# hvasbath/beat

Measured on AMD Instinct MI355X. Metric: SMC chain-steps/s (FFI seismic gfstacking 400 patches x 64 targets x 4096 samples), higher is better.
Workload: dtype f64; 1 GPU; BASELINE configs[2]: FFI seismic gfstacking, 400 patches x 64 targets x 4096 samples, library (64,400,3,25,4096) f64 = 62.9 GB in HBM, nearest_neighbor, covariance scalar; population SURVEY 8(d): nucleation U over the 20x20 fault, time 0; chains_per_gpu=512, global_chains=512, parallelism=chains sharded over 1 GPU(s), library replicated

## Files before the change

### beat_amd/csrc/ctx.hpp

```cpp
#pragma once
#include <hip/hip_runtime.h>

#include <cstdarg>
#include <cstdint>
#include <cstdio>
#include <cstring>
#include <map>
#include <memory>
#include <string>
#include <vector>

#include "../../include/beat_amd.h"

struct beatamd_ctx;

namespace beatamd {

void set_error(const char *fmt, ...);

#define BA_HIP(expr)                                                                         \
    do {                                                                                     \
        hipError_t e_ = (expr);                                                              \
        if (e_ != hipSuccess) {                                                              \
            beatamd::set_error("%s:%d: %s -> %s", __FILE__, __LINE__, #expr,                 \
// ... 170 lines not shown
    std::vector<int64_t> sizes;
    std::vector<int32_t> wsets;
    DevMem<int64_t> hp_off;
    bool corr_set = false;
    GeoCorr corr;
    DevMem<GeoCorrTerm> corr_terms;
    DevMem<double> corr_basis;
    DevMem<PoleTerm> pole_terms;
    mutable DevMem<double> pole_coef;
    mutable int64_t pole_chains = 0;
};

struct GeomSources {
    int nsrc = 0;
    DevMem<int32_t> kind;
    DevMem<int64_t> poff;
    DevMem<double> pfix;
    DevMem<double> east, north, los;
    int64_t Nobs = 0;
    double nu = 0.25;
};

constexpr int POL_MTQT = 0, POL_MT = 1, POL_DC = 2;
constexpr int POL_MAX_MAPS = 8;
struct PolSource {
    int32_t kind = POL_MTQT, pad_ = 0;
    int64_t off[6] = {-1, -1, -1, -1, -1, -1};
    double fix[6] = {0, 0, 0, 0, 0, 0};
};
struct Polarity {
    PolSource src;
    int32_t nmap = 0;
    int64_t NT = 0;
    int64_t map_end[POL_MAX_MAPS] = {};
    int64_t hp_off[POL_MAX_MAPS] = {};
    double hp_fix[POL_MAX_MAPS] = {};
    double gamma = 0.2;
    DevMem<double> rw, obs;
    int32_t ntab = 0;
    DevMem<double> utab, btab;
};

struct FfiModel {
    beatamd_ffi_layout layout;
    int32_t nsub = 0;
    std::vector<int32_t> ndip, nstrike, patch_off;
    std::vector<double> patch_size;
    int64_t P = 0;
    DevMem<int32_t> d_ndip, d_nstrike, d_patch_off;
    DevMem<double> d_patch_size;
    std::vector<Wavemap> wavemaps;
    bool has_geo = false;
    Geodetic geo;
    bool geo_is_geometry = false;
    GeomSources geom;
    bool has_pol = false;
    Polarity pol;
    int32_t lap = -1;
    int64_t nllk() const;
    bool obs_quads_valid = false;
    std::vector<double> obs_quads;
    DevMem<double> d_obs_quads;
    int32_t lsq_var = -1, lsq_zero_var = -1;
    bool lsq_blocks_valid = false;
    DevMem<double> lsq_GG, lsq_LtL;
};

struct HyperModel {
    int64_t nterm = 0, nh = 0;
    DevMem<double> M, slog;
    DevMem<int32_t> kind, hp_index;
    int32_t ngroups = 0, group_end[8] = {0, 0, 0, 0, 0, 0, 0, 0};
};

constexpr int KNOB_UNSET = -2147483647;
#define BEATAMD_GF_KNOBS(X) \
    X(gf_kernel, "BEATAMD_GF_KERNEL") X(gs_cg, "BEATAMD_GS_CG") X(gs_ws, "BEATAMD_GS_WS") X(gs_dma, "BEATAMD_GS_DMA") X(gs_nt, "BEATAMD_GS_NT") \
    X(ws_map, "BEATAMD_WS_MAP") X(gs_pair, "BEATAMD_GS_PAIR") X(gs_nthint, "BEATAMD_GS_NTHINT") X(gs_order, "BEATAMD_GS_ORDER") \
    X(gs_fit, "BEATAMD_GS_FIT") X(gs_win, "BEATAMD_GS_WIN") X(gf_tinv, "BEATAMD_GF_TINV") X(gs_tune, "BEATAMD_GS_TUNE") \
    X(gf_order, "BEATAMD_GF_ORDER") X(gf_cgroup, "BEATAMD_GF_CGROUP") X(gs_ml, "BEATAMD_GS_ML") X(gc_global, "BEATAMD_GC_GLOBAL") \
    X(gc_sort, "BEATAMD_GC_SORT") X(gc_keys, "BEATAMD_GC_KEYS") X(gc_bands, "BEATAMD_GC_BANDS") X(gr_cap, "BEATAMD_GR_CAP") \
    X(gr_pass_alloc, "BEATAMD_GR_PASS_ALLOC") X(gr_var, "BEATAMD_GR_VAR") X(sweep_v1, "BEATAMD_SWEEP_V1") X(qf_band, "BEATAMD_QF_BAND") \
    X(qf_fuse, "BEATAMD_QF_FUSE") X(gf_split, "BEATAMD_GF_SPLIT") X(gm_wave, "BEATAMD_GM_WAVE") X(skip_parked, "BEATAMD_SKIP_PARKED") \
    X(td_strip, "BEATAMD_TD_STRIP") X(pd_strip, "BEATAMD_PD_STRIP") X(pd_rows, "BEATAMD_PD_ROWS")
struct GfKnobs {
#define X(member, env) int member = KNOB_UNSET;
    BEATAMD_GF_KNOBS(X)
#undef X
    void read_env();
    static int get(int v, int dflt) { return v == KNOB_UNSET ? dflt : v; }
    static bool is(int v, int x) { return v != KNOB_UNSET && v == x; }
    static bool set(int v) { return v != KNOB_UNSET; }
};

struct KTimer {
    double total_ms = 0;
    int64_t n = 0;
    std::vector<std::pair<hipEvent_t, hipEvent_t>> pending;
};

}

struct beatamd_ctx {
    int device = 0;
    hipStream_t stream = nullptr, own_stream = nullptr;
    bool timing = false;
    std::map<std::string, beatamd::KTimer> timers;
    std::vector<hipEvent_t> event_pool;
    int *d_status = nullptr;
    std::vector<beatamd::DevBuf> scratch_bufs;
    std::vector<std::unique_ptr<beatamd::SeisStore>> seislibs;
    std::vector<std::unique_ptr<beatamd::GeoLib>> geolibs;
    std::vector<std::unique_ptr<beatamd::GeoEnsemble>> geoens;
    std::vector<std::unique_ptr<beatamd::WeightSet>> wsets;
    std::vector<std::unique_ptr<beatamd::Laplacian>> laps;
    std::vector<std::unique_ptr<beatamd::FfiModel>> models;
    std::vector<std::unique_ptr<beatamd::HyperModel>> hypers;
    int num_cu = 256;
    char last_gf_kernel[96] = "";
    int64_t gs_ngtp = 0, gs_N = 0;
    double gs_trep = 1;
    int gs_nvar = 1;
    bool gs_has_passes = false;
    char gf_plan[384] = "";
    char gf_tune_log[512] = "";
    uint32_t *h_umax = nullptr;
    hipEvent_t umax_event = nullptr;
    bool umax_pending = false;
    int umax_hist = -1, umax_hist_cg = 0;
    std::map<std::vector<int64_t>, std::pair<int, int>> gs_tuned;
    int gs_cg = 0;
    beatamd::GfKnobs knobs;
    bool knobs_live = false;
    uint32_t *step_dev = nullptr;
    std::map<int64_t, beatamd::DevMem<double>> twiddles;

    int get_scratch(int slot, size_t bytes, void **out);
    template <class T>
    int scratch(int slot, size_t n, T **out)
    {
        void *raw = nullptr;
        const int rc = get_scratch(slot, n * sizeof(T), &raw);
        *out = static_cast<T *>(raw);
        return rc;
    }
    hipEvent_t get_event();
    void time_begin(const char *name);
    void time_end(const char *name);
    int check_status();
};

namespace beatamd {

bool is_device_ptr(const void *p);
const GfKnobs &gf_knobs(beatamd_ctx *ctx);

enum Slot : int {
    SL_IN0 = 0, SL_IN1, SL_IN2, SL_IN3, SL_IN4, SL_IN5, SL_IN6, SL_IN7,
    SL_OUT0, SL_OUT1, SL_OUT2, SL_OUT3, SL_OUT4, SL_OUT5, SL_OUT6, SL_OUT7,
    SL_ROWOFF, SL_WEIGHTS, SL_ST0, SL_RESID, SL_PARTIAL, SL_PARTIAL2, SL_QUAD, SL_MU, SL_SLIPS,
    SL_QPROP, SL_LPROP, SL_MISC, SL_GS_UROWS, SL_GS_UCOUNT, SL_GS_SLOT, SL_GS_W, SL_GS_UMAX, SL_GS_USLOT,
    SL_CHAINBAD, SL_Z, SL_ROWSCALE, SL_CUM, SL_STAGE2, SL_WHITEN,
    SL_CHOL_A, SL_CHOL_X, SL_CHOL_D, SL_CHOL_T, SL_CHOL_L,
    SL_GC_ORDER, SL_GS_ORDER, SL_GC_STREAM, SL_GC_HDR, SL_GC_META, SL_DELTA, SL_LOGU, SL_EDGES, SL_TSLOT, SL_SPLIT, SL_WS_PACK,
    SL_GM_W, SL_GM_SCALE, SL_GM_FLAG, SL_LSQ_N, SL_LSQ_B, SL_LSQ_X, SL_LSQ_U, SL_MR_SPANS,
    SL_RES_GG, SL_RES_N, SL_RES_W, SL_RES_T, SL_RES_U, SL_RATE_DMIN, SL_SPEC,
    SL_MG_FLAG, SL_MG_MOM, SL_MG_PAR, SL_MG_GRID, SL_MG_W, SL_MG_BOX,
    SL_MC_FLAG, SL_MC_COUNT, SL_MC_SUM, SL_PD_BOX,
    SL_CV_W, SL_CV_SA, SL_CV_SB, SL_CV_Q, SL_CV_CM, SL_CV_RM, SL_CV_OFF, SL_CV_ESS, SL_CV_ACT, SL_CV_STATE, SL_CV_MAC0, SL_CV_MAC1,
    SL_CV_AC, SL_CV_RHO, SL_CV_PART, SL_COUNT
};
constexpr int SL_NIN = SL_OUT0 - SL_IN0, SL_NOUT = SL_ROWOFF - SL_OUT0;

class Staging {
    beatamd_ctx *ctx;
    int nin = 0, nout = 0, nback = 0;
    struct { void *host, *dev; size_t bytes; } back[SL_NOUT];
    int in_bytes(const void *p, size_t bytes, const void **dev);
    int out_bytes(void *p, size_t bytes, void **dev, bool preload);

public:
    explicit Staging(beatamd_ctx *c) : ctx(c) {}
    template <class T>
    int in(const T *p, size_t n, const T **dev)
    {
        const void *d = nullptr;
        BA_TRY(in_bytes(p, n * sizeof(T), &d));
        *dev = static_cast<const T *>(d);
        return BEATAMD_OK;
    }
    template <class T>
    int out(T *p, size_t n, T **dev, bool preload = false)
    {
        void *d = nullptr;
        BA_TRY(out_bytes(p, n * sizeof(T), &d, preload));
        *dev = static_cast<T *>(d);
        return BEATAMD_OK;
    }
    int finish();
};

struct ScopedTimer {
    beatamd_ctx *c;
    const char *n;
    ScopedTimer(beatamd_ctx *ctx, const char *name) : c(ctx), n(name) { c->time_begin(n); }
    ~ScopedTimer() { c->time_end(n); }
};

}
```

### beat_amd/csrc/gfshared.hip

```cpp
#include "kernels.hpp"
#include "misfit.hpp"
#include "wave.hpp"

namespace beatamd {

constexpr int GS_NT_MAX = 64;
constexpr int GS_NTHINT_DEFAULT = 1;
constexpr int GS_WS_DEFAULT = 1;

struct GroupTabArgs {
    int nrow, nvar, CG;
    int64_t C, T, P, DS;
    const uint32_t *rowoff;
    const double *fac;
    ChainVec slips[4];
    int ucap, ustride;
    uint32_t *urows;
    uint32_t *uent;
    int nissue;
    int windowed;
    int depth;
    uint32_t *ucount;
    uint32_t *umax;
    uint16_t *slot;
// ... 1441 lines not shown
    *ucap_out = (int)std::max<int64_t>(ucap, 2);
    return true;
}

GfGroup gfstack_group(const GfPlan &p, int cg, int ucap)
{
    GfGroup g;
    g.cg = cg; g.ucap = ucap;
    g.ws = p.ws512 && cg == WS_CG;
    g.mode = p.mode;
    if (p.mode == GF_RESID_BAND1) g.band1 = gf_band1(g.ws && !p.f32 && !p.pair64 && p.fused, GF_BY_WS, &g.mode);
    return g;
}

bool gfstack_shared_plan(const GfStackCall &k, GfPlan &p)
{
    const SeisLib &L = *k.libs[0];
    if (L.N % 2 != 0) return false;
    const GfKnobs &kn = *p.knobs;
    if (GfKnobs::is(kn.gf_kernel, 0)) return false;
    if (!GfKnobs::is(kn.gf_kernel, 1) && k.C < 48) return false;
    p.ws512 = GfKnobs::get(kn.gs_ws, GS_WS_DEFAULT) != 0 && k.interp != BEATAMD_MULTILINEAR && L.N % 2 == 0 &&
              !(GfKnobs::set(kn.gs_dma) && kn.gs_dma != 2) && !(GfKnobs::set(kn.gs_nt) && kn.gs_nt != 64);
    int cg = pick_group(k.C);
    const int gq = GfKnobs::get(kn.gs_cg, 0);
    if (gq == 64 || gq == 128 || gq == 256 || gq == 512 || gq == 1024) cg = gq;
    if (p.R > 1) {
        if (!p.ws512) return false;
        cg = WS_CG;
    }
    const bool ws = p.ws512 && cg == WS_CG;
    while (!ws && std::min<int64_t>((int64_t)cg * p.nrow, L.D * L.S) * (GS_NT_MAX + 2) * 8 > 72 * 1024 && cg > 64) cg /= 2;
    int ucap = 0;
    if (!shared_fit(k, p, cg, ws, &ucap)) return false;
    p.group = gfstack_group(p, cg, ucap);
    p.tune = !GfKnobs::set(kn.gs_cg) && !GfKnobs::is(kn.gs_tune, 0);
    const int cand[4] = {512, 256, 128, 64};
    for (int i = 0; i < 4 && p.tune; i++) {
        if (p.R > 1 && cand[i] != 512) continue;
        if (cand[i] > 64 && (int64_t)cand[i] / 2 >= k.C) continue;
        if (k.C >= 1024 && cand[i] < 256) continue;
        if (k.C >= 384 && cand[i] < 128) continue;
        int u = 0;
        if (shared_fit(k, p, cand[i], p.ws512 && cand[i] == WS_CG, &u)) p.cand[p.ncand++] = gfstack_group(p, cand[i], u);
    }
    return true;
}

static void gs_common_args(GsArgs &a, const GfStackCall &k, const GfPlan &p, const GfLaunch &ln, int64_t ngroups)
{
    const GfKnobs &kn = *p.knobs;
    const SeisLib &L = *k.libs[0];
    memset(&a, 0, sizeof(a));
    for (int v = 0; v < k.nvar; v++) {
        a.G[v] = k.libs[v]->g;
        a.G32[v] = k.libs[v]->g32;
    }
    a.nvar = k.nvar;
    a.C = k.C; a.T = L.T; a.P = L.P; a.N = L.N;
    a.Ttab = p.Ttab; a.rows_per_target = L.P * L.D * L.S;
    a.tslot = ln.tslot;
    a.ngroups = ngroups;
    a.data = k.data; a.wscalar = k.wscalar; a.out = k.out;
    a.nthint = GfKnobs::set(kn.gs_nthint) ? (kn.gs_nthint != 0) : (GS_NTHINT_DEFAULT && ngroups == 1);
}

static int64_t gs_grid(GsArgs &a, const GfKnobs &kn)
{
    a.xcd_order = (a.ngroups > 1 && !GfKnobs::is(kn.gs_order, 0)) ? 1 : 0;
    if (GfKnobs::is(kn.gs_order, 1)) a.xcd_order = 1;
    return a.xcd_order ? ((a.T * a.ntile + 7) / 8) * 8 * a.ngroups : a.ngroups * a.T * a.ntile;
}

void gs_record_stats(beatamd_ctx *ctx, const GfStackCall &k, int64_t GTP, int64_t Ttab, int cg, bool has_passes)
{
    ctx->gs_ngtp = GTP;
    ctx->gs_trep = (double)k.libs[0]->T / (double)Ttab;
    ctx->gs_N = k.libs[0]->N;
    ctx->gs_cg = cg;
    ctx->gs_nvar = k.nvar;
    ctx->gs_has_passes = has_passes;
}

static int launch_gfstack_ws(beatamd_ctx *ctx, const GfStackCall &k, const GfPlan &p, const GfLaunch &ln, const GfGroup &g)
{
    const GfKnobs &kn = *p.knobs;
    const SeisLib &L = *k.libs[0];
    const int64_t Ttab = p.Ttab;
    const int mode = g.mode;
    const int64_t ngroups = (k.C + WS_CG - 1) / WS_CG;
    const int64_t GT = ngroups * Ttab, GTP = GT * L.P;
    const int64_t bound = std::min<int64_t>(WS_CG, L.D * L.S);
    const int cap = bound <= 32 ? 32 : bound <= 64 ? 64 : WS_CAP_MAX;
    const int maxpass = (int)((bound + cap - 1) / cap);
    const int64_t vmax = L.P * maxpass;

    WsTabArgs ta;
    memset(&ta, 0, sizeof(ta));
    ta.nvar = k.nvar; ta.cap = cap;
    ta.C = k.C; ta.T = Ttab; ta.P = L.P; ta.DS = L.D * L.S; ta.vmax = vmax;
    ta.rowoff = ln.rowoff;
    for (int v = 0; v < k.nvar; v++) ta.slips[v] = k.slips[v];
    ta.R = p.R;
    if (ngroups > 1 && k.order_key[0].base && k.order_key[1].base && GfKnobs::get(kn.gc_global, 1) != 0)
        BA_TRY(launch_chain_members(ctx, k.C, k.order_key, WS_CG, ngroups, &ta.order, GfKnobs::get(kn.gc_global, 1) == 2));
    BA_TRY(ctx->scratch(SL_GS_UCOUNT, (size_t)(3 * GTP + GT), &ta.utotal));
    ta.npass = ta.utotal + GTP;
    uint32_t *voff = ta.npass + GTP, *nv = voff + GTP;
    const size_t nvs = (size_t)GT * vmax + 3;
    BA_TRY(ctx->scratch(SL_GS_UROWS, nvs, &ta.ucount));
    BA_TRY(ctx->scratch(SL_GS_USLOT, nvs * WS_USTRIDE * 2, &ta.uent));
    BA_TRY(ctx->scratch(SL_GS_SLOT, nvs * WS_CG, &ta.slot));
    ta.w_var_stride = (int64_t)GT * vmax * WS_CG;
    BA_TRY(ctx->scratch(SL_GS_W, (size_t)ta.w_var_stride * k.nvar + (size_t)3 * WS_CG, &ta.w));
    {
        ScopedTimer tm(ctx, "grouptables");
        if (k.active) {
            uint32_t *packed;
            BA_TRY(ctx->scratch(SL_WS_PACK, (size_t)ngroups * WS_CG, &packed));
            hipLaunchKernelGGL(k_ws_pack, dim3((unsigned)ngroups), dim3(WS_CG), 0, ctx->stream, ta.order, k.active, k.C, packed);
            ta.order = packed;
        }
        const bool map = ta.DS <= WS_MAP_MAX && !GfKnobs::is(kn.ws_map, 0);
        const size_t mlds = map ? (size_t)ta.DS * sizeof(uint16_t) : 0;
        if (maxpass > 1) {
            if (map) hipLaunchKernelGGL((k_ws_tables<0, 1>), dim3((unsigned)GTP), dim3(WS_CG), mlds, ctx->stream, ta);
            else hipLaunchKernelGGL((k_ws_tables<0, 0>), dim3((unsigned)GTP), dim3(WS_CG), 0, ctx->stream, ta);
            hipLaunchKernelGGL(k_ws_scan, dim3((unsigned)GT), dim3(256), 0, ctx->stream, ta.npass, voff, nv, L.P);
            ta.voff = voff;
        }
        if (map) hipLaunchKernelGGL((k_ws_tables<1, 1>), dim3((unsigned)GTP), dim3(WS_CG), mlds, ctx->stream, ta);
        else hipLaunchKernelGGL((k_ws_tables<1, 0>), dim3((unsigned)GTP), dim3(WS_CG), 0, ctx->stream, ta);
    }
    BA_HIP(hipGetLastError());

    GsArgs a;
    const bool f32 = p.f32, pair64 = p.pair64;
    gs_common_args(a, k, p, ln, ngroups);
    a.nrow = 1;
    a.CG = WS_CG; a.ucap = cap; a.ustride = WS_USTRIDE;
    a.nt = 64; a.dma = 2; a.ws = 3;
    a.ntile = (int)((L.N + 63) / 64);
    a.nv = maxpass > 1 ? nv : nullptr;
    a.vmax = vmax;
    a.order = ta.order;
    a.uent = ta.uent; a.ucount = ta.ucount; a.slot = ta.slot; a.w = ta.w;
    a.w_var_stride = ta.w_var_stride;
    if (mode == GF_RESID_SCALAR || mode == GF_RESID_BAND1) BA_TRY(ctx->scratch(SL_PARTIAL, (size_t)k.C * L.T * a.ntile, &a.partial));
    if (mode == GF_RESID_BAND1) {
        BA_TRY(ctx->scratch(SL_EDGES, (size_t)k.C * L.T * a.ntile * 2, &a.edges));
        a.band_w = k.band_w;
    }
    const int64_t nblocks = gs_grid(a, kn);
    BA_CHECK(nblocks < (int64_t)0x7fffffff, BEATAMD_EINVAL, "gfstack: batch too large");
    size_t lds = f32 ? (size_t)(cap + 1) * (64 + 2) * sizeof(float) * 3
                     : (size_t)(cap + 1) * (64 + (pair64 ? 2 : 1)) * sizeof(double) * 3;
    lds = std::max<size_t>(lds, (64 + 8 * 64 * 17) * sizeof(double));
    BA_CHECK(lds <= 160 * 1024, BEATAMD_EINVAL, "internal: k_gfstack_ws row buffers exceed LDS");
    if (f32 || pair64)
        snprintf(ctx->last_gf_kernel, sizeof(ctx->last_gf_kernel), "k_gfstack_ws%s<%d,%d,%d>", f32 ? "32" : "p64", mode, a.ws,
                 a.nthint);
    else
        snprintf(ctx->last_gf_kernel, sizeof(ctx->last_gf_kernel), "k_gfstack_ws<%d,%d,%d,%d>", 1, mode, a.ws, a.nthint);
    snprintf(ctx->gf_plan, sizeof(ctx->gf_plan),
             "loader/consumer kernel: 512-chain groups, nearest neighbour; %d row slots per LDS buffer (a patch can touch min(512, "
             "D*S = %lld) rows), %s", cap, (long long)(L.D * L.S),
             maxpass > 1 ? "patches that touch more are staged in passes of equal size" : "one pass per patch");
    gs_record_stats(ctx, k, GTP, Ttab, WS_CG, maxpass > 1);
    {
        ScopedTimer tm(ctx, "gfstack");
        BA_TRY(launch_ws(mode, dim3((unsigned)nblocks), lds, ctx->stream, a, f32 ? 1 : (pair64 ? 2 : 0)));
    }
    BA_HIP(hipGetLastError());
    if (a.partial)
        BA_TRY(launch_sum_tiles(ctx, a.partial, k.C * L.T, a.ntile, k.quad, nullptr, 0, a.edges, k.band_w, L.T, L.N));
    return BEATAMD_OK;
}

static int launch_dma_twin(beatamd_ctx *ctx, const GfStackCall &k, const GfPlan &p, const GfGroup &g, GsArgs &shared, int twin,
                           int ucap, bool windowed, int64_t GTP)
{
    const SeisLib &L = *k.libs[0];
    const int nrow = p.nrow, CG = g.cg, mode = g.mode;
    GsArgs a = shared;
    a.ucap = ucap;
    a.guard_mode = twin;
    size_t lds = (size_t)ucap * (a.nt + 2) * sizeof(double);
    BA_CHECK(2 * lds <= 158 * 1024, BEATAMD_EINVAL, "internal: k_gfstack_dma row buffers exceed LDS");
    a.dma = GfKnobs::is(p.knobs->gs_dma, 1) ? 1 : 2;
    if (a.nt == 32 && a.dma != 2) { a.nt = 64; a.ntile = (int)((L.N + 63) / 64); lds = (size_t)ucap * (a.nt + 2) * sizeof(double); }
    BA_CHECK(CG != 1024 || a.dma == 2, BEATAMD_EINVAL, "gfstack: 1024-chain groups need the LDS-DMA kernel");
    BA_CHECK(!windowed || a.dma == 2, BEATAMD_EINVAL, "internal: window slots need the ds_read_b64 kernel");
    a.ws = 0;
    a.f32pair = 0;
    if (a.dma == 2 && a.nt == 64 && CG <= 512 && p.f32) {
        a.f32pair = 1;
        lds = std::max<size_t>((size_t)ucap * (a.nt + 2) * sizeof(float) * 2, 64 * sizeof(double));
    } else {
        lds *= 2;
    }
    const dim3 grid((unsigned)gs_grid(a, *p.knobs));
    if (a.f32pair)
        snprintf(ctx->last_gf_kernel, sizeof(ctx->last_gf_kernel), "k_gfstack_dmaf<%d,%d,%d>", CG / 64, nrow, mode);
    else
        snprintf(ctx->last_gf_kernel, sizeof(ctx->last_gf_kernel), "%s<%d,%d,%d,%d,%d>",
                 "k_gfstack_dma", CG / 64, nrow, mode, a.nt, a.dma == 2 ? 1 : 0);
    gs_record_stats(ctx, k, GTP, p.Ttab, CG, false);
    snprintf(ctx->gf_plan, sizeof(ctx->gf_plan),
             "lane <-> chain kernel with %d-chain groups (%s): row buffers of %d slots%s", CG,
             k.C < 384 ? "small batch" : nrow == 4 ? "multilinear below 192 chains or an odd sample count" : "group size measured fastest",
             ucap, twin ? " sized by the previous launch's distinct-row count" : "");
    if (CG == 1024) BA_TRY(launch_shared_nrow<16>(nrow, mode, grid, lds, ctx->stream, a));
    else if (CG == 512) BA_TRY(launch_shared_nrow<8>(nrow, mode, grid, lds, ctx->stream, a));
    else if (CG == 256) BA_TRY(launch_shared_nrow<4>(nrow, mode, grid, lds, ctx->stream, a));
    else if (CG == 128) BA_TRY(launch_shared_nrow<2>(nrow, mode, grid, lds, ctx->stream, a));
    else BA_TRY(launch_shared_nrow<1>(nrow, mode, grid, lds, ctx->stream, a));
    BA_HIP(hipGetLastError());
    shared.nt = a.nt; shared.ntile = a.ntile;
    return BEATAMD_OK;
}

int launch_gfstack_shared(beatamd_ctx *ctx, const GfStackCall &k, const GfPlan &p, const GfLaunch &ln, const GfGroup &g)
{
    if (g.ws) return launch_gfstack_ws(ctx, k, p, ln, g);
    const GfKnobs &kn = *p.knobs;
    const SeisLib &L = *k.libs[0];
    const int nrow = p.nrow, CG = g.cg, mode = g.mode;
    int ucap = g.ucap;
    const int64_t Ttab = p.Ttab;
    const int64_t ngroups = (k.C + CG - 1) / CG;
    const int64_t GTP = ngroups * Ttab * L.P;

    GroupTabArgs ga;
    memset(&ga, 0, sizeof(ga));
    ga.nrow = nrow; ga.nvar = k.nvar; ga.CG = CG;
    ga.C = k.C; ga.T = Ttab; ga.P = L.P; ga.DS = L.D * L.S;
    ga.rowoff = ln.rowoff; ga.fac = ln.fac;
    for (int v = 0; v < k.nvar; v++) ga.slips[v] = k.slips[v];
    ga.ucap = ucap;
    ga.ustride = (ucap + 63) / 64 * 64;
    BA_TRY(ctx->scratch(SL_GS_UROWS, (size_t)GTP * ga.ustride, &ga.urows));
    BA_TRY(ctx->scratch(SL_GS_USLOT, (size_t)GTP * ga.ustride * 2, &ga.uent));
    BA_TRY(ctx->scratch(SL_GS_UCOUNT, (size_t)GTP, &ga.ucount));
    BA_TRY(ctx->scratch(SL_GS_SLOT, (size_t)(GTP + 3) * nrow * CG, &ga.slot));
    ga.w_var_stride = (nrow == 1) ? ngroups * L.P * CG : GTP * 4 * CG;
    BA_TRY(ctx->scratch(SL_GS_W, (size_t)ga.w_var_stride * k.nvar + (size_t)3 * 4 * CG, &ga.w));
    const bool fit_lds = CG <= 128 && !GfKnobs::is(kn.gs_fit, 0);
    if (fit_lds) {
        BA_TRY(ctx->scratch(SL_GS_UMAX, 1, &ga.umax));
        BA_HIP(hipMemsetAsync(ga.umax, 0, sizeof(uint32_t), ctx->stream));
    }
    ga.nissue = CG / 64;
    {
        const int depth = (ucap + 31) / 32;
        const bool dma2 = !(GfKnobs::is(kn.gs_dma, 0) || GfKnobs::is(kn.gs_dma, 1)) && L.N % 2 == 0;
        ga.windowed = (CG >= 512 && nrow == 1 && dma2 && ucap > 32 && ucap <= 128 && !GfKnobs::is(kn.gs_win, 0) &&
                       (size_t)2 * 32 * depth * (GS_NT_MAX + 2) * 8 <= 158 * 1024) ? 1 : 0;
        ga.depth = depth;
        if (ga.windowed) ucap = 32 * depth;
    }
    {
        ScopedTimer tm(ctx, "grouptables");
        const size_t lds = (size_t)(2 * ga.DS + CG + 1 + 256) * sizeof(uint32_t);
        hipLaunchKernelGGL(k_gf_group_tables, dim3((unsigned)GTP), dim3(CG), lds, ctx->stream, ga);
    }
    BA_HIP(hipGetLastError());

    GsArgs a;
    gs_common_args(a, k, p, ln, ngroups);
    a.nrow = nrow;
    a.CG = CG; a.ucap = ucap; a.ustride = ga.ustride;
    a.nt = GfKnobs::is(kn.gs_nt, 32) || CG == 1024 ? 32 : 64;
    a.ntile = (int)((L.N + a.nt - 1) / a.nt);
    a.urows = ga.urows; a.uent = ga.uent; a.ucount = ga.ucount; a.slot = ga.slot; a.w = ga.w;
    a.w_var_stride = ga.w_var_stride;
    if (mode == GF_RESID_SCALAR) BA_TRY(ctx->scratch(SL_PARTIAL, (size_t)k.C * L.T * a.ntile, &a.partial));
    BA_CHECK(ngroups * L.T * a.ntile < (int64_t)0x7fffffff, BEATAMD_EINVAL, "gfstack: batch too large");
    int ucap_fit = 0;
    if (fit_lds) {
        if (!ctx->h_umax) {
            BA_HIP(hipHostMalloc((void **)&ctx->h_umax, sizeof(uint32_t), hipHostMallocDefault));
            BA_HIP(hipEventCreateWithFlags(&ctx->umax_event, hipEventDisableTiming));
        }
        hipStreamCaptureStatus cap = hipStreamCaptureStatusNone;
        BA_HIP(hipStreamIsCapturing(ctx->stream, &cap));
        const bool capturing = cap != hipStreamCaptureStatusNone;
        if (!capturing && ctx->umax_pending && hipEventQuery(ctx->umax_event) == hipSuccess) {
            ctx->umax_hist = (int)*ctx->h_umax;
            ctx->umax_pending = false;
        }
        (void)hipGetLastError();
        if (ctx->umax_hist >= 0 && ctx->umax_hist_cg == CG && a.nt == 64) {
            const int want = ctx->umax_hist + 1;
            if (want < ucap) ucap_fit = std::max(want, 2);
        }
        if (!capturing && !ctx->umax_pending) {
            BA_HIP(hipMemcpyAsync(ctx->h_umax, ga.umax, sizeof(uint32_t), hipMemcpyDeviceToHost, ctx->stream));
            BA_HIP(hipEventRecord(ctx->umax_event, ctx->stream));
            ctx->umax_pending = true;
            ctx->umax_hist_cg = CG;
        }
    }
    a.guard_fit = ucap_fit;
    a.guard_umax = ga.umax;
    ScopedTimer tm(ctx, "gfstack");
    if (ucap_fit) BA_TRY(launch_dma_twin(ctx, k, p, g, a, 1, ucap_fit, ga.windowed, GTP));
    BA_TRY(launch_dma_twin(ctx, k, p, g, a, ucap_fit ? 2 : 0, ucap, ga.windowed, GTP));
    if (mode == GF_RESID_SCALAR) BA_TRY(launch_sum_tiles(ctx, a.partial, k.C * L.T, a.ntile, k.quad));
    return BEATAMD_OK;
}

}
```

### beat_amd/csrc/gfstack.hip

```cpp
#include <cstdlib>
#include <cstring>

#include "kernels.hpp"
#include "misfit.hpp"

namespace beatamd {

struct TabArgs {
    int interp;
    int64_t C, T, P, D, S;
    double st_min, st_dt, du_min, du_dt;
    ChainVec durations;
    StartTimeSrc st;
    uint32_t *rowoff;
    double *fac;
    int *status;
    int64_t R;
};

__device__ __forceinline__ int to_int16(double x) { return (int)(int16_t)(long long)x; }

__device__ __forceinline__ bool wrap_index(int &i, int n)
{
    if (i < 0) i += n;
    return i >= 0 && i < n;
}

__global__ void __launch_bounds__(256) k_gf_tables(TabArgs a)
{
    const int64_t idx = (int64_t)blockIdx.x * 256 + threadIdx.x;
    const int64_t total = a.C * a.T * a.P;
    if (idx >= total) return;
    const int64_t p = idx % a.P;
    const int64_t ct = idx / a.P;
    const int64_t t = ct % a.T;
    const int64_t c = ct / a.T;

    const int64_t ts = t / a.R, pr = (t % a.R) * a.P + p, Preal = a.P * a.R;
    double st;
    if (a.st.explicit_st) {
        st = a.st.explicit_st[(c * (a.T / a.R) + ts) * Preal + pr];
    } else {
        st = a.st.starttimes0[c * Preal + pr];
        if (a.st.shift_off) st = st - a.st.Q[c * a.st.nparams + a.st.shift_off[ts]];
    }
    const double du = a.durations.base[c * a.durations.stride + a.durations.off + pr];
    const int D = (int)a.D, S = (int)a.S;
    const int64_t row0 = (t * a.P + p) * a.D;
    bool ok = true;
    if (a.interp == BEATAMD_NEAREST_NEIGHBOR) {
        int si = to_int16(rint((st - a.st_min) / a.st_dt));
        int di = to_int16(rint((du - a.du_min) / a.du_dt));
        const bool ok_s = wrap_index(si, S), ok_d = wrap_index(di, D);
        ok = ok_s && ok_d;
        if (!ok) { si = 0; di = 0; }
        a.rowoff[idx] = (uint32_t)((row0 + di) * a.S + si);
    } else {
        const double ds = (st - a.st_min) / a.st_dt;
        const double dd = (du - a.du_min) / a.du_dt;
        int sc = to_int16(ceil(ds)), dc = to_int16(ceil(dd));
        const double stf = (double)sc - ds, rtf = (double)dc - dd;
        int sf = sc - 1, df = dc - 1;
        const bool o1 = wrap_index(sc, S), o2 = wrap_index(dc, D), o3 = wrap_index(sf, S),
                   o4 = wrap_index(df, D);
        ok = o1 && o2 && o3 && o4;
        if (!ok) { sc = dc = sf = df = 0; }
        uint32_t *ro = a.rowoff + idx * 4;
        double *fa = a.fac + idx * 4;
        ro[0] = (uint32_t)((row0 + dc) * a.S + sc);
        ro[1] = (uint32_t)((row0 + dc) * a.S + sf);
        ro[2] = (uint32_t)((row0 + df) * a.S + sc);
        ro[3] = (uint32_t)((row0 + df) * a.S + sf);
        fa[0] = (1 - stf) * (1 - rtf);
        fa[1] = stf * (1.0 - rtf);
        fa[2] = (1 - stf) * rtf;
        fa[3] = stf * rtf;
    }
    if (!ok) {
        atomicOr(a.status, ST_INDEX_OOB);
        if (a.st.chain_bad) a.st.chain_bad[c] = 1;
    }
}

struct GfArgs {
    const double *G[4];
    ChainVec slips[4];
    int64_t T, P, N;
    const uint32_t *rowoff;
    const double *fac;
    const double *data;
    const double *wscalar;
    double *out;
    double *partial;
    int ntile;
    int order;
    int64_t C;
    int cgroup;
    int64_t Ttab, rows_per_target;
    const int32_t *tslot;
    const int *guard;
    int64_t nblocks;
    int64_t R;
};

template <int W> struct VecT;
template <> struct VecT<2> { using type = double2; };
template <> struct VecT<1> { using type = double; };

template <int W>
__device__ __forceinline__ typename VecT<W>::type ldg(const double *p)
{
    return *reinterpret_cast<const typename VecT<W>::type *>(p);
}
__device__ __forceinline__ void fma_acc(double2 &acc, double2 x, double w)
{
    acc.x = fma(x.x, w, acc.x);
    acc.y = fma(x.y, w, acc.y);
}
__device__ __forceinline__ void fma_acc(double &acc, double x, double w) { acc = fma(x, w, acc); }

template <int INTERP, int NVAR, int VEC, int W, int MODE>
__device__ __forceinline__ void gfstack_tile(const GfArgs &a, const int64_t bid)
{
    using V = typename VecT<W>::type;
    constexpr int NROW = INTERP ? 4 : 1;
    constexpr int CH = 256 * W;
    constexpr int U = (8 / (NROW * NVAR * VEC)) > 0 ? (8 / (NROW * NVAR * VEC)) : 1;

    const int tile = (int)(bid % a.ntile);
    const int64_t bq = bid / a.ntile;
    int64_t c, t;
    if (a.order == 0) {
        c = bq / a.T;
        t = bq - c * a.T;
    } else {
        const int64_t per_group = (int64_t)a.cgroup * a.T;
        const int64_t g = bq / per_group;
        const int64_t r = bq - g * per_group;
        const int64_t c0 = g * a.cgroup;
// ... 66 lines not shown
#pragma unroll
                for (int v = 0; v < VEC; v++) fma_acc(acc[v], ldg<W>(row + n[v]), w);
            }
        }
    }

    if (MODE == GF_STORE_SYN) {
#pragma unroll
        for (int v = 0; v < VEC; v++)
            if (inb[v]) *reinterpret_cast<V *>(a.out + ct * N + n[v]) = acc[v];
    } else if (MODE == GF_RESID_STORE) {
#pragma unroll
        for (int v = 0; v < VEC; v++)
            if (inb[v]) {
                V d = ldg<W>(a.data + t * N + n[v]);
                V r;
                if constexpr (W == 2) { r.x = d.x - acc[v].x; r.y = d.y - acc[v].y; }
                else { r = d - acc[v]; }
                *reinterpret_cast<V *>(a.out + ct * N + n[v]) = r;
            }
    } else {
        const double w = a.wscalar[t];
        double q = 0.0;
#pragma unroll
        for (int v = 0; v < VEC; v++)
            if (inb[v]) {
                V d = ldg<W>(a.data + t * N + n[v]);
                if constexpr (W == 2) {
                    double t0 = w * (d.x - acc[v].x), t1 = w * (d.y - acc[v].y);
                    q = fma(t0, t0, q);
                    q = fma(t1, t1, q);
                } else {
                    double t0 = w * (d - acc[v]);
                    q = fma(t0, t0, q);
                }
            }
        for (int off = 32; off > 0; off >>= 1) q += __shfl_down(q, off, 64);
        __shared__ double red[4];
        if ((threadIdx.x & 63) == 0) red[threadIdx.x >> 6] = q;
        __syncthreads();
        if (threadIdx.x == 0)
            a.partial[ct * a.ntile + tile] = ((red[0] + red[1]) + red[2]) + red[3];
    }
}

template <int INTERP, int NVAR, int VEC, int W, int MODE>
__global__ void __launch_bounds__(256) k_gfstack(GfArgs a)
{
    if (a.guard) {
        if (*a.guard == 0) return;
        for (int64_t b = blockIdx.x; b < a.nblocks; b += gridDim.x) {
            gfstack_tile<INTERP, NVAR, VEC, W, MODE>(a, b);
            __syncthreads();
        }
    } else {
        gfstack_tile<INTERP, NVAR, VEC, W, MODE>(a, blockIdx.x);
    }
}

__global__ void __launch_bounds__(256) k_round_to_f32(double *g, float *g32, int64_t n)
{
    for (int64_t i = (int64_t)blockIdx.x * 256 + threadIdx.x; i < n; i += (int64_t)gridDim.x * 256) {
        const float f = (float)g[i];
        g32[i] = f;
        g[i] = (double)f;
    }
}

int launch_round_to_f32(beatamd_ctx *ctx, double *g, float *g32, int64_t n)
{
    if (n == 0) return BEATAMD_OK;
    const unsigned grid = (unsigned)std::min<int64_t>((n + 255) / 256, 1 << 20);
    hipLaunchKernelGGL(k_round_to_f32, dim3(grid), dim3(256), 0, ctx->stream, g, g32, n);
    BA_HIP(hipGetLastError());
    return BEATAMD_OK;
}

__global__ void __launch_bounds__(256) k_sum_tiles(const double *partial, int64_t n, int ntile, double *quad, const int *guard,
                                                  int want, const double *edges, const double *band_w, int64_t T, int64_t N)
{
    const int64_t i = (int64_t)blockIdx.x * 256 + threadIdx.x;
    if (i >= n) return;
    if (guard_skips(guard, want)) return;
    const int64_t t = edges ? i % T : 0;
    double s = 0.0;
    for (int k = 0; k < ntile; k++) {
        if (edges && k + 1 < ntile) {
            const double *w = band_w + (t * N + (int64_t)k * 64 + 63) * 2;
            const double *e = edges + (i * ntile + k) * 2;
            s = band1_join(s, partial[i * ntile + k], true, w[0], w[1], e[1], e[2]);
        } else {
            s = tile_join(s, partial[i * ntile + k]);
        }
    }
    quad[i] = s;
}

int launch_sum_tiles(beatamd_ctx *ctx, const double *partial, int64_t n, int ntile, double *quad, const int *guard, int want,
                     const double *edges, const double *band_w, int64_t T, int64_t N)
{
    hipLaunchKernelGGL(k_sum_tiles, dim3((unsigned)((n + 255) / 256)), dim3(256), 0, ctx->stream, partial, n, ntile, quad,
                       guard, want, edges, band_w, T, N);
    BA_HIP(hipGetLastError());
    return BEATAMD_OK;
}

template <int INTERP, int NVAR, int VEC, int W>
static void launch_mode(int mode, dim3 grid, hipStream_t s, const GfArgs &a)
{
    if (mode == GF_STORE_SYN)
        hipLaunchKernelGGL((k_gfstack<INTERP, NVAR, VEC, W, GF_STORE_SYN>), grid, dim3(256), 0, s, a);
    else if (mode == GF_RESID_SCALAR)
        hipLaunchKernelGGL((k_gfstack<INTERP, NVAR, VEC, W, GF_RESID_SCALAR>), grid, dim3(256), 0, s, a);
    else
        hipLaunchKernelGGL((k_gfstack<INTERP, NVAR, VEC, W, GF_RESID_STORE>), grid, dim3(256), 0, s, a);
}

template <int INTERP, int VEC, int W>
static void launch_nvar(int nvar, int mode, dim3 grid, hipStream_t s, const GfArgs &a)
{
    if (nvar == 1) launch_mode<INTERP, 1, VEC, W>(mode, grid, s, a);
    else if (nvar == 2) launch_mode<INTERP, 2, VEC, W>(mode, grid, s, a);
    else launch_mode<INTERP, 3, VEC, W>(mode, grid, s, a);
}

static int launch_gfstack_impl(beatamd_ctx *ctx, const GfStackCall &call, const GfPlan &p, GfLaunch &ln);

int gf_patch_ranges(int64_t T, int64_t P, int64_t N, int num_cu)
{
    if (N > 256 || P < 64) return 1;
    const int64_t walks = T * ((N + 63) / 64);
    const int64_t ncu = std::max(1, num_cu);
    if (walks >= 2 * ncu) return 1;
    int best = 1;
    int64_t best_cost = ((walks + ncu - 1) / ncu) * (P + 5);
    for (int d = 2; d <= 32 && P / d >= 32; d++) {
        if (P % d) continue;
        const int64_t cost = ((walks * d + ncu - 1) / ncu) * (P / d + 5);
        if (cost < best_cost) { best = d; best_cost = cost; }
    }
    return best;
}

__global__ void __launch_bounds__(256) k_split_tslot(int64_t Tv, int R, const int32_t *tslot, int32_t *out)
{
    const int64_t t = (int64_t)blockIdx.x * 256 + threadIdx.x;
    if (t < Tv) out[t] = (tslot ? tslot[t / R] : 0) * R + (int32_t)(t % R);
}

template <int MODE>
__global__ void __launch_bounds__(256) k_split_combine(const double *part, int64_t C, int64_t T, int64_t N, int R,
                                                      const double *data, const double *wscalar, double *out, double *quad,
                                                      const double *band_w)
{
    __shared__ double sq[256 + 1];
    __shared__ double tsum[4];
    const int64_t ct = blockIdx.x, t = ct % T, c = ct / T;
    const int n = threadIdx.x;
    double v = 0.0;
    if (n < N) {
        const double *pp = part + ((c * T + t) * R) * N + n;
        double syn = pp[0];
        for (int r = 1; r < R; r++) syn += pp[(int64_t)r * N];
        if (MODE == GF_STORE_SYN) out[ct * N + n] = syn;
        else if (MODE == GF_RESID_SCALAR) v = scalar_t(wscalar[t], data[t * N + n], syn);
        else if (MODE == GF_RESID_BAND1) v = data[t * N + n] - syn;
        else out[ct * N + n] = data[t * N + n] - syn;
    }
    if (MODE != GF_RESID_SCALAR && MODE != GF_RESID_BAND1) return;
    sq[n] = v;
    __syncthreads();
    const int ntile = (int)((N + 63) / 64);
    const int n0 = n * 64, nv = (int)min((int64_t)64, N - (int64_t)n0);
    __shared__ double w[MODE == GF_RESID_BAND1 ? 2 * 256 : 2];
    if (MODE == GF_RESID_BAND1) {
        if (n < N) {
            w[2 * n] = band_w[(t * N + n) * 2];
            w[2 * n + 1] = band_w[(t * N + n) * 2 + 1];
        }
        __syncthreads();
    }
    if (n < ntile) {
        const auto r = [&](int i) { return sq[n0 + i]; };
        if (MODE == GF_RESID_BAND1) tsum[n] = band1_tile<false, 64>(r, [&](int i, int b) { return w[2 * (n0 + i) + b]; }, nv, n0 + nv == N).q;
        else tsum[n] = scalar_tile<false, 64>(r, nv);
    }
    __syncthreads();
    if (n == 0) {
        double s_ = 0.0;
        for (int k = 0; k < ntile; k++) {
            const int last = k * 64 + 63;
            if (MODE == GF_RESID_BAND1 && k + 1 < ntile) s_ = band1_join(s_, tsum[k], true, w[2 * last], w[2 * last + 1], sq[last], sq[last + 1]);
            else s_ = tile_join(s_, tsum[k]);
        }
        quad[ct] = s_;
    }
}

GfPlan gf_plan_call(const GfStackCall &k, const GfKnobs &kn, int num_cu)
{
    GfPlan p;
    const SeisLib &L = *k.libs[0];
    p.knobs = &kn;
    const int split = GfKnobs::get(kn.gf_split, -1);
    p.R = split == 0 || split == 1 ? 1 : split > 1 ? ((L.P % split == 0 && L.N <= 256) ? split : 1)
                                   : gf_patch_ranges(L.split_T > 0 ? L.split_T : L.T, L.P, L.N, num_cu);
    p.T = L.T * p.R; p.P = L.P / p.R;
    p.tinv = !k.st.explicit_st && !k.st.shift_off && !GfKnobs::is(kn.gf_tinv, 0);
    p.slots = !k.st.explicit_st && k.st.shift_off && k.st.nslot > 0 && !GfKnobs::is(kn.gf_tinv, 0);
    p.Ttab = p.tinv ? p.R : p.slots ? (int64_t)k.st.nslot * p.R : p.T;
    p.nrow = k.interp == BEATAMD_MULTILINEAR ? 4 : 1;
    p.f32 = k.f32;
    for (int v = 0; v < k.nvar; v++) p.f32 = p.f32 && k.libs[v]->g32 != nullptr;
    p.pair64 = GfKnobs::is(kn.gs_pair, 1);
    p.fused = !GfKnobs::is(kn.qf_fuse, 0);
    p.mode = p.R > 1 ? (int)GF_STORE_SYN : k.mode;
    p.mode_combine = k.mode;
    if (p.R > 1 && k.mode == GF_RESID_BAND1) p.band1 = gf_band1(p.fused, GF_BY_COMBINE, &p.mode_combine);
    const bool band1 = p.mode == GF_RESID_BAND1;
    p.mode_standin = band1 ? (int)GF_RESID_STORE : p.mode;
    if (!p.f32 && gfstack_ml_applicable(k, p)) {
        p.stacker = GF_RUNS;
        p.standin_band1 = band1 && p.fused;
        if (band1) p.band1 = gf_band1(p.fused, GF_BY_RUNS, &p.mode);
    } else if (gfstack_shared_plan(k, p)) {
        p.stacker = GF_GROUPS;
    } else if (band1) {
        p.band1 = gf_band1(false, GF_BY_NONE, &p.mode);
    }
    return p;
}

static int tune_group_size(beatamd_ctx *ctx, const GfStackCall &k, const GfPlan &p, const GfLaunch &ln, GfGroup *out)
{
    const SeisLib &L = *k.libs[0];
    const int64_t cbucket = k.C < 512 ? k.C : 512 * std::min<int64_t>((k.C + 511) / 512, 16);
    const std::vector<int64_t> key = {cbucket, p.nrow, k.nvar, L.T, L.P, L.D, L.S, L.N, p.Ttab, p.f32 ? 1 : 0};
    auto it = ctx->gs_tuned.find(key);
    if (it == ctx->gs_tuned.end()) {
        const int nc = p.ncand;
        int best = -1;
        float best_ms = 0.f, ms_of[4] = {0.f, 0.f, 0.f, 0.f};
        hipEvent_t e0, e1;
        BA_HIP(hipEventCreate(&e0)); BA_HIP(hipEventCreate(&e1));
        for (int i = 0; i < nc && nc > 1; i++) {
            float ms_min = 0.f;
            for (int rep = 0; rep < 2; rep++) {
                BA_HIP(hipEventRecord(e0, ctx->stream));
                BA_TRY(launch_gfstack_shared(ctx, k, p, ln, p.cand[i]));
                BA_HIP(hipEventRecord(e1, ctx->stream));
                BA_HIP(hipEventSynchronize(e1));
                BA_HIP(hipEventElapsedTime(&ms_min, e0, e1));
            }
            ms_of[i] = ms_min;
            if (best < 0 || ms_min < best_ms) { best = i; best_ms = ms_min; }
            if (ms_min > 2.f * best_ms) break;
        }
        (void)hipEventDestroy(e0); (void)hipEventDestroy(e1);
        if (nc == 1) best = 0;
        if (best >= 0) it = ctx->gs_tuned.emplace(key, std::make_pair(p.cand[best].cg, p.cand[best].ucap)).first;
        char *w = ctx->gf_tune_log; size_t left = sizeof(ctx->gf_tune_log);
        int n = snprintf(w, left, "group size for %lld chains (T %lld, P %lld, D*S %lld, N %lld, %d row(s) per chain): ",
                         (long long)k.C, (long long)L.T, (long long)L.P, (long long)(L.D * L.S), (long long)L.N, p.nrow);
        for (int i = 0; i < nc && n > 0 && (size_t)n < left; i++) {
            w += n; left -= (size_t)n;
            n = ms_of[i] > 0.f ? snprintf(w, left, "%d: %.3f ms%s", p.cand[i].cg, ms_of[i], i + 1 < nc ? ", " : "")
                               : snprintf(w, left, "%d: %s%s", p.cand[i].cg, nc == 1 ? "only candidate" : "not timed", i + 1 < nc ? ", " : "");
        }
        if (best >= 0 && n > 0 && (size_t)n < left) { w += n; left -= (size_t)n; snprintf(w, left, " -> %d", p.cand[best].cg); }
        if (getenv("BEATAMD_VERBOSE")) fprintf(stderr, "beat_amd: %s\n", ctx->gf_tune_log);
    }
    *out = it != ctx->gs_tuned.end() ? gfstack_group(p, it->second.first, it->second.second) : p.group;
    return BEATAMD_OK;
}

static int launch_gfstack_split(beatamd_ctx *ctx, const GfStackCall &call, const GfPlan &p, GfLaunch &ln)
{
    const SeisLib &L = *call.libs[0];
    const int R = p.R;
    SeisLib views[4];
    GfStackCall v = call;
    v.active = nullptr;
    for (int i = 0; i < call.nvar; i++) {
        views[i] = *call.libs[i];
        views[i].T = p.T; views[i].P = p.P;
        v.libs[i] = &views[i];
    }
    double *part;
    BA_TRY(ctx->scratch(SL_SPLIT, (size_t)call.C * L.T * R * L.N, &part));
    v.out = part;
    v.quad = nullptr; v.data = nullptr; v.wscalar = nullptr; v.band_w = nullptr;
    BA_TRY(launch_gfstack_impl(ctx, v, p, ln));
    const size_t n0 = strlen(ctx->gf_plan);
    snprintf(ctx->gf_plan + n0, sizeof(ctx->gf_plan) - n0, "; %lld-sample traces: patches stacked in %d ranges of %lld "
             "(%lld walks instead of %lld), partial synthetics summed in range order", (long long)L.N, R, (long long)(L.P / R),
             (long long)(L.T * R * ((L.N + 63) / 64)), (long long)(L.T * ((L.N + 63) / 64)));
    const dim3 grid((unsigned)(call.C * L.T));
    BA_CHECK(call.C * L.T < (int64_t)0x7fffffff, BEATAMD_EINVAL, "gfstack: batch too large");
    ScopedTimer tm(ctx, "gfcombine");
    const int mode = p.mode_combine;
    const auto combine = mode == GF_STORE_SYN ? k_split_combine<GF_STORE_SYN> : mode == GF_RESID_SCALAR ? k_split_combine<GF_RESID_SCALAR>
                       : mode == GF_RESID_BAND1 ? k_split_combine<GF_RESID_BAND1> : k_split_combine<GF_RESID_STORE>;
    hipLaunchKernelGGL(combine, grid, dim3(256), 0, ctx->stream, part, call.C, L.T, L.N, R, call.data, call.wscalar, call.out,
                       call.quad, mode == GF_RESID_BAND1 ? call.band_w : (const double *)nullptr);
    BA_HIP(hipGetLastError());
    return BEATAMD_OK;
}

int launch_gfstack(beatamd_ctx *ctx, const GfStackCall &call)
{
    const SeisLib &L = *call.libs[0];
    BA_CHECK(call.nvar >= 1 && call.nvar <= 3, BEATAMD_EINVAL, "gfstack: 1..3 slip variables supported");
    for (int v = 1; v < call.nvar; v++) {
        const SeisLib &M = *call.libs[v];
        BA_CHECK(M.T == L.T && M.P == L.P && M.D == L.D && M.S == L.S && M.N == L.N && M.st_min == L.st_min && M.st_dt == L.st_dt &&
                     M.du_min == L.du_min && M.du_dt == L.du_dt,
                 BEATAMD_EINVAL, "gfstack: libraries of the slip variables differ in shape/grid");
    }
    BA_CHECK(L.T * L.P * L.D * L.S < (int64_t)0xffffffffLL, BEATAMD_EINVAL, "gfstack: library has more than 2^32 rows");
    const GfPlan p = gf_plan_call(call, gf_knobs(ctx), ctx->num_cu);
    GfLaunch ln;
    if (p.R > 1) {
        BA_TRY(launch_gfstack_split(ctx, call, p, ln));
    } else {
        if (call.mode == GF_RESID_BAND1)
            BA_CHECK(call.band_w && call.quad && call.out && call.data, BEATAMD_EINVAL, "gfstack: mode 3 needs band_w, quad, out, data");
        BA_TRY(launch_gfstack_impl(ctx, call, p, ln));
    }
    if ((p.stacker == GF_GROUPS && p.R == 1 ? ln.group.band1 : p.band1) == GF_BY_QUADFORM)
        BA_TRY(launch_quadform_banded(ctx, call.band_w, 1, L.N, L.T, call.C, call.out, L.T * L.N, L.N, call.quad, L.T));
    return BEATAMD_OK;
}

static int launch_gfstack_impl(beatamd_ctx *ctx, const GfStackCall &k, const GfPlan &p, GfLaunch &ln)
{
    const GfKnobs &kn = *p.knobs;
    const SeisLib &L = *k.libs[0];
    if (k.C == 0) return BEATAMD_OK;
    const int64_t R = p.R, Ttab = p.Ttab;
    ln.tslot = p.slots ? k.st.tslot : nullptr;
    if (R > 1 && (p.tinv || p.slots)) {
        int32_t *vslot;
        BA_TRY(ctx->scratch(SL_TSLOT, (size_t)L.T, &vslot));
        hipLaunchKernelGGL(k_split_tslot, dim3((unsigned)((L.T + 255) / 256)), dim3(256), 0, ctx->stream, L.T, (int)R,
                           p.slots ? k.st.tslot : nullptr, vslot);
        ln.tslot = vslot;
    }
    const int64_t CTP = k.C * Ttab * L.P;

    TabArgs ta;
    ta.interp = k.interp; ta.R = R;
    ta.C = k.C; ta.T = Ttab; ta.P = L.P; ta.D = L.D; ta.S = L.S;
    ta.st_min = L.st_min; ta.st_dt = L.st_dt; ta.du_min = L.du_min; ta.du_dt = L.du_dt;
    ta.durations = k.durations; ta.st = k.st;
    if (p.slots) ta.st.shift_off = k.st.slot_shift_off;
    ta.status = ctx->d_status;
    BA_TRY(ctx->scratch(SL_ROWOFF, (size_t)CTP * p.nrow, &ta.rowoff));
    ta.fac = nullptr;
    if (p.nrow == 4) BA_TRY(ctx->scratch(SL_WEIGHTS, (size_t)CTP * 4, &ta.fac));
    {
        ScopedTimer tm(ctx, "tables");
        hipLaunchKernelGGL(k_gf_tables, dim3((unsigned)((CTP + 255) / 256)), dim3(256), 0,
                           ctx->stream, ta);
    }
    BA_HIP(hipGetLastError());
    ln.rowoff = ta.rowoff; ln.fac = ta.fac;

    const int *standin = nullptr;
    if (p.stacker == GF_RUNS) {
        BA_TRY(launch_gfstack_ml(ctx, k, p, ln, &standin));
        if (!standin) return BEATAMD_OK;
    } else if (p.stacker == GF_GROUPS) {
        ln.group = p.group;
        if (p.tune) BA_TRY(tune_group_size(ctx, k, p, ln, &ln.group));
        return launch_gfstack_shared(ctx, k, p, ln, ln.group);
    }
    const int mode = standin ? p.mode_standin : p.mode;

    GfArgs a;
    memset(&a, 0, sizeof(a));
    for (int v = 0; v < k.nvar; v++) {
        a.G[v] = k.libs[v]->g;
        a.slips[v] = k.slips[v];
    }
    a.T = L.T; a.P = L.P; a.N = L.N;
    a.Ttab = Ttab; a.rows_per_target = L.P * L.D * L.S;
    a.tslot = ln.tslot;
    a.C = k.C;
    a.R = R;
    a.order = GfKnobs::get(kn.gf_order, 1);
    a.cgroup = std::max(1, GfKnobs::get(kn.gf_cgroup, 128));
    a.rowoff = ta.rowoff; a.fac = ta.fac;
    a.data = k.data; a.wscalar = k.wscalar; a.out = k.out;
    a.guard = standin;
    const int W = (L.N % 2 == 0) ? 2 : 1;
    const int VEC = 1;
    const int64_t tile_w = (int64_t)256 * W * VEC;
    a.ntile = (int)((L.N + tile_w - 1) / tile_w);
    if (mode == GF_RESID_SCALAR) BA_TRY(ctx->scratch(standin ? SL_PARTIAL2 : SL_PARTIAL, (size_t)k.C * L.T * a.ntile, &a.partial));
    const int64_t nblocks = k.C * L.T * a.ntile;
    BA_CHECK(nblocks < (int64_t)0x7fffffff, BEATAMD_EINVAL, "gfstack: batch too large (%lld blocks)",
             (long long)nblocks);
    a.nblocks = nblocks;
    dim3 grid((unsigned)(standin ? std::min<int64_t>(nblocks, (int64_t)ctx->num_cu * 8) : nblocks));
    if (!standin) {
        snprintf(ctx->last_gf_kernel, sizeof(ctx->last_gf_kernel), "k_gfstack<%d,%d,%d,%d,%d>",
                 k.interp == BEATAMD_MULTILINEAR ? 1 : 0, k.nvar, VEC, W, mode);
        snprintf(ctx->gf_plan, sizeof(ctx->gf_plan), "streaming kernel: %s", k.C < 48 ? "fewer than 48 chains share too few rows" :
                 L.N % 2 ? "odd sample count (the chain-shared kernels move 16-byte lanes)" : "chosen by BEATAMD_GF_KERNEL or no chain-shared kernel fits this library");
        ctx->gs_ngtp = 0;
    }
    {
        ScopedTimer tm(ctx, standin ? "gfstack_standin" : "gfstack");
        const auto launch = k.interp == BEATAMD_NEAREST_NEIGHBOR ? (W == 2 ? launch_nvar<0, 1, 2> : launch_nvar<0, 1, 1>)
                                                                 : (W == 2 ? launch_nvar<1, 1, 2> : launch_nvar<1, 1, 1>);
        launch(k.nvar, mode, grid, ctx->stream, a);
    }
    BA_HIP(hipGetLastError());
    if (mode == GF_RESID_SCALAR) BA_TRY(launch_sum_tiles(ctx, a.partial, k.C * L.T, a.ntile, k.quad, standin, 1));
    if (standin && p.standin_band1)
        BA_TRY(launch_quadform_banded(ctx, k.band_w, 1, L.N, L.T, k.C, k.out, L.T * L.N, L.N, k.quad, L.T, standin, 1));
    return BEATAMD_OK;
}

int launch_gf_tables(beatamd_ctx *ctx, const GfStackCall &k, uint32_t *rowoff, double *fac)
{
    const SeisLib &L = *k.libs[0];
    if (k.C == 0) return BEATAMD_OK;
    BA_CHECK(L.T * L.P * L.D * L.S < (int64_t)0xffffffffLL, BEATAMD_EINVAL, "gfstack: library has more than 2^32 rows");
    BA_CHECK(rowoff && (k.interp != BEATAMD_MULTILINEAR || fac), BEATAMD_EINVAL, "gf_tables: bad argument");
    const int64_t CTP = k.C * L.T * L.P;
    BA_CHECK((CTP + 255) / 256 < (int64_t)0x7fffffff, BEATAMD_EINVAL, "gf_tables: batch too large");
    TabArgs ta;
    ta.interp = k.interp; ta.R = 1;
    ta.C = k.C; ta.T = L.T; ta.P = L.P; ta.D = L.D; ta.S = L.S;
    ta.st_min = L.st_min; ta.st_dt = L.st_dt; ta.du_min = L.du_min; ta.du_dt = L.du_dt;
    ta.durations = k.durations; ta.st = k.st;
    ta.status = ctx->d_status;
    ta.rowoff = rowoff; ta.fac = fac;
    ScopedTimer tm(ctx, "tables");
    hipLaunchKernelGGL(k_gf_tables, dim3((unsigned)((CTP + 255) / 256)), dim3(256), 0, ctx->stream, ta);
    BA_HIP(hipGetLastError());
    return BEATAMD_OK;
// ... 4 lines not shown
```

### beat_amd/csrc/kernels.hpp

```cpp
#pragma once
#include <algorithm>

#include "ctx.hpp"

namespace beatamd {

constexpr int SWEEP_MAX_CELLS = 6400;
struct SweepLdsPlan {
    int nmax;
    int waves;
    size_t bytes;
};
SweepLdsPlan sweep_lds_plan(int nmax_cells);
int launch_sweep_explicit(beatamd_ctx *ctx, const double *slow, double h, const int32_t *hi,
                          const int32_t *hj, int ni, int nj, int64_t C, double *out);
int launch_sweep_model(beatamd_ctx *ctx, const FfiModel &m, const double *Q, int64_t C,
                       double *starttimes0, int32_t *chain_bad);

struct StartTimeSrc {
    const double *explicit_st = nullptr;
    const double *starttimes0 = nullptr;
    const double *Q = nullptr;
    int64_t nparams = 0;
    const int64_t *shift_off = nullptr;
    int32_t nslot = 0;
    const int32_t *tslot = nullptr;
    const int64_t *slot_shift_off = nullptr;
    int32_t *chain_bad = nullptr;
};

struct ChainVec {
    const double *base = nullptr;
    int64_t stride = 0, off = 0;
};

#ifdef __HIPCC__
__device__ __forceinline__ int64_t xcd_items8(int64_t b, int64_t n)
{
    if (b >= (n & ~(int64_t)63)) return b;
    const int64_t r = b & 63;
    return (b & ~(int64_t)63) + (r & 7) * 8 + (r >> 3);
}
#endif

int gf_patch_ranges(int64_t T, int64_t P, int64_t N, int num_cu);

enum GfMode : int {
    GF_STORE_SYN = 0,
    GF_RESID_SCALAR = 1,
    GF_RESID_STORE = 2,
    GF_RESID_BAND1 = 3
};

struct GfStackCall {
    const SeisLib *libs[4] = {nullptr, nullptr, nullptr, nullptr};
    int nvar = 1;
    ChainVec slips[4];
    ChainVec durations;
    StartTimeSrc st;
    int interp = 0;
    int64_t C = 0;
    int mode = GF_STORE_SYN;
    const double *data = nullptr;
    const double *wscalar = nullptr;
    double *out = nullptr;
    double *quad = nullptr;
    const double *band_w = nullptr;
    bool f32 = false;
    ChainVec order_key[2];
    const int32_t *active = nullptr;
};
int launch_gfstack(beatamd_ctx *ctx, const GfStackCall &call);
int launch_sum_tiles(beatamd_ctx *ctx, const double *partial, int64_t n, int ntile, double *quad, const int *guard = nullptr,
                     int want = 0, const double *edges = nullptr, const double *band_w = nullptr, int64_t T = 1, int64_t N = 0);
int launch_round_to_f32(beatamd_ctx *ctx, double *g, float *g32, int64_t n);
enum GfBand1 : int { GF_BY_NONE, GF_BY_COMBINE, GF_BY_RUNS, GF_BY_WS, GF_BY_QUADFORM };
inline GfBand1 gf_band1(bool carries, GfBand1 by, int *mode)
{
    if (!carries) *mode = GF_RESID_STORE;
    return carries ? by : GF_BY_QUADFORM;
}
enum GfStacker : int { GF_STREAMING, GF_RUNS, GF_GROUPS };
struct GfGroup {
    int cg = 0, ucap = 0, mode = 0;
    bool ws = false;
    GfBand1 band1 = GF_BY_NONE;
};
struct GfPlan {
    const GfKnobs *knobs = nullptr;
    int R = 1;
    int64_t T = 0, P = 0;
    bool tinv = false, slots = false;
    int64_t Ttab = 0;
    int nrow = 1;
    bool f32 = false, pair64 = false, fused = true, ws512 = false;
    GfStacker stacker = GF_STREAMING;
    int mode = 0, mode_standin = 0, mode_combine = 0;
    bool standin_band1 = false;
    GfBand1 band1 = GF_BY_NONE;
    GfGroup group, cand[4];
    int ncand = 0;
    bool tune = false;
};
GfPlan gf_plan_call(const GfStackCall &call, const GfKnobs &kn, int num_cu);
struct GfLaunch {
    const int32_t *tslot = nullptr;
    const uint32_t *rowoff = nullptr;
    const double *fac = nullptr;
    GfGroup group;
};
void gs_record_stats(beatamd_ctx *ctx, const GfStackCall &k, int64_t GTP, int64_t Ttab, int cg, bool has_passes);
bool gfstack_shared_plan(const GfStackCall &call, GfPlan &p);
GfGroup gfstack_group(const GfPlan &p, int cg, int ucap);
int launch_gfstack_shared(beatamd_ctx *ctx, const GfStackCall &call, const GfPlan &p, const GfLaunch &ln, const GfGroup &g);

int launch_chain_members(beatamd_ctx *ctx, int64_t C, const ChainVec key[2], int64_t cg, int64_t ngroups, const uint32_t **members,
                         int strips = 0);
bool gfstack_ml_applicable(const GfStackCall &call, const GfPlan &p);
int launch_gfstack_ml(beatamd_ctx *ctx, const GfStackCall &call, const GfPlan &p, const GfLaunch &ln, const int **ovf);

struct QuadformCall {
    const double *A = nullptr;
    int64_t a_stride = 0;
    int64_t M = 0, nd = 0, C = 0;
    const double *X = nullptr;
    int64_t xs_c = 0, xs_d = 0;
    int upper_tri = 0;
    double *quad = nullptr;
    int64_t q_stride = 0;
};
int launch_quadform(beatamd_ctx *ctx, const QuadformCall &call);
constexpr int QF_BAND_LIMIT = 16;
int launch_band_detect(beatamd_ctx *ctx, const double *A, int64_t nd, int64_t M, void *scratch, int64_t *band_host,
                       double *dropped_rel_host);
int launch_band_pack(beatamd_ctx *ctx, const double *A, int64_t nd, int64_t M, int64_t band, double *wb);
int launch_quadform_banded(beatamd_ctx *ctx, const double *wb, int64_t band, int64_t M, int64_t nd, int64_t C, const double *X,
                           int64_t xs_c, int64_t xs_d, double *quad, int64_t q_stride, const int *guard = nullptr, int want = 0);
struct QuadformSmallCall {
    int nd = 0;
    const double *A[8];
    int64_t M[8], xoff[8];
    int upper_tri[8];
    const double *slog[8];
    const int64_t *hp_off[8];
    int64_t C = 0;
    const double *X = nullptr;
    int64_t xs_c = 0;
    const double *Q = nullptr;
    int64_t nparams = 0;
    double *LL = nullptr;
    int64_t ld = 0;
    bool misfit_only = false;
};
bool quadform_small_applicable(int nd, const int64_t *M);
// ... 86 lines not shown
#pragma clang fp contract(off)
    const double r = (d - mu) * odw;
    const int c0 = __builtin_amdgcn_readfirstlane((int)c);
    if (__all(c == (int64_t)c0))
        return geo_corr_subtract<true>(gc, Q + (int64_t)c0 * nparams, gc.pole + (int64_t)c0 * gc.pole_stride, k, r);
    return geo_corr_subtract<false>(gc, Q + c * nparams, gc.pole + c * gc.pole_stride, k, r);
}
#endif
int launch_store_misfits(beatamd_ctx *ctx, int64_t C, int64_t n, const double *src, double *dst, int64_t ld);
int launch_misfits_mark_bad(beatamd_ctx *ctx, int64_t C, int64_t n, double *llks, const int32_t *chain_bad);
int launch_laplacian_finish(beatamd_ctx *ctx, int64_t C, int64_t nvar, int64_t P, double logdet,
                            const double *quad, HpSrc hp, double *out, int64_t ld);
struct LikeGroups {
    int32_t end[8];
    int n = 0;
};
int launch_like_sum(beatamd_ctx *ctx, int64_t C, int64_t nllk, const LikeGroups &grp, double *LL,
                    const int32_t *chain_bad);
int launch_like_assemble(beatamd_ctx *ctx, int64_t C, int64_t nllk, int64_t nsrc, const double *src, const int32_t *dst_col,
                         const double *rest, int64_t rest_ld, int64_t rest_col0, int64_t n_rest, int64_t rest_dst0,
                         const LikeGroups &grp, double *LL, int32_t *chain_bad);
int launch_gather_slips(beatamd_ctx *ctx, int64_t C, int nvar, int64_t P, const ChainVec *slips,
                        double *out);
int launch_geom_los(beatamd_ctx *ctx, const GeomSources &g, const double *Q, int64_t nparams,
                    int64_t C, double *mu, const double *data = nullptr, const double *odw = nullptr,
                    double *res = nullptr, GeoCorr gc = GeoCorr());
int launch_geom_disp(beatamd_ctx *ctx, int nsrc, const int32_t *kind, const int64_t *poff,
                     const double *params, int64_t C, int64_t nobs, const double *east,
                     const double *north, double nu, double *out);
int launch_geo_gf_library(beatamd_ctx *ctx, int64_t nrows, const double *params, const int32_t *kind,
                          const int64_t *poff, int64_t nobs, const double *east, const double *north,
                          const double *los, const double *odw, double nu, double *G);
int launch_smoothing_correlated(beatamd_ctx *ctx, int64_t P, const double *coords, int kind, double *L);
int launch_model_resolution(beatamd_ctx *ctx, int64_t P, int64_t nobs, const double *gfs, const double *L,
                            double epsilon, double *R, double *diag);
int launch_division_rating(beatamd_ctx *ctx, int64_t P, int64_t nobs, const double *widths, const double *lengths,
                           const double *centers, const double *bottom_depth, double depth_penalty,
                           const double *data_en, const double *mean_R, double *dmin, double *rating);
int launch_autocovariance(beatamd_ctx *ctx, int64_t nd, int64_t n, const double *data,
                          const double *mean, double *out);
int launch_scaled_toeplitz(beatamd_ctx *ctx, int64_t nd, int64_t n, const double *coeffs,
                           const double *stds, double *out);


struct GemmCall {
    const double *A = nullptr, *B = nullptr, *row_scale = nullptr;
    double *O = nullptr;
    int64_t lda = 0, ldb = 0, ldo = 0, M = 0, N = 0, K = 0;
    int b_kn = 0;
    int b_upper = 0;
    const char *timer = nullptr;
    int nbatch = 1;
    int64_t sA = 0, sB = 0, sO = 0;
    int64_t sR = 0;
    double alpha = 1.0;
    int accumulate = 0;
    int lower_only = 0;
    int b_lower = 0;
    int col_block = -1;
};
int launch_gemm_f64(beatamd_ctx *ctx, const GemmCall &call);
int launch_chol_inverse(beatamd_ctx *ctx, int64_t nbatch, int64_t n, const double *C, double *W, double *log_pdet,
                        int32_t *notpsd = nullptr);
int launch_gram_cholesky(beatamd_ctx *ctx, int64_t K, int64_t n, const double *F, double *R);
int launch_triu_ratio(beatamd_ctx *ctx, int64_t nbatch, int64_t n, const double *Wn, const double *Wo, double *M);
int launch_potrf_lower(beatamd_ctx *ctx, int64_t nbatch, int64_t np, double *A, int32_t *notpsd);
int launch_triu_solve_vec(beatamd_ctx *ctx, int64_t nbatch, int64_t n, const double *W, double *X);

int launch_smc_calc_beta(beatamd_ctx *ctx, int64_t n, const double *lik, int64_t stride, double beta,
                         double cv, int mode, double dbeta, double *out2, double *weights);
int launch_smc_resample(beatamd_ctx *ctx, int64_t n, const double *weights, double aux, double *cum,
                        int32_t *idx);
int launch_pop_factor(beatamd_ctx *ctx, int64_t n, int64_t np, const double *X, int64_t ldx,
                      const double *w, double *F);
int launch_gather_rows(beatamd_ctx *ctx, int64_t nout, int64_t ncol, const double *src, int64_t lds,
                       int64_t nrow_src, const int32_t *idx, double *out, int64_t ldo);
int launch_tune_scaling(beatamd_ctx *ctx, int64_t C, double *scaling, int32_t *accepted, double interval);
int launch_accumulate_i32(beatamd_ctx *ctx, int64_t C, const int32_t *a, int32_t *acc);
int launch_philox_normal(beatamd_ctx *ctx, double *z, int64_t C, int64_t K, uint64_t seed,
                         uint32_t step, uint64_t first_chain);
int launch_philox_univariate(beatamd_ctx *ctx, double *delta, int64_t C, int64_t np, int kind,
                             const double *scale, uint64_t seed, uint32_t step, uint64_t first_chain);
int launch_step_advance(beatamd_ctx *ctx);
bool draw_propose_applicable(int64_t K, int64_t np);
int launch_draw_propose(beatamd_ctx *ctx, int64_t C, int64_t K, int64_t np, int kind, const double *factor,
                        int df, uint64_t seed, uint32_t step, uint64_t first_chain, const double *Q0,
                        const double *scaling, const double *lower, const double *upper, double *Qprop,
                        double *log_u, int32_t *inbounds, int64_t groups = 1);
int launch_philox_chain(beatamd_ctx *ctx, int64_t C, uint64_t seed, uint32_t step, uint64_t first_chain,
                        int df, double *log_u, double *row_scale);
int launch_propose(beatamd_ctx *ctx, int64_t C, int64_t nparams, const double *Q0,
                   const double *delta, const double *scaling, const double *lower,
                   const double *upper, double *Qprop, int32_t *inbounds);
int launch_accept(beatamd_ctx *ctx, int64_t C, int64_t nparams, int64_t nllk, double *Q0,
                  double *L0, const double *Qprop, double *Lprop, const int32_t *inbounds,
                  const double *log_u, double beta, const double *betas, int32_t *accepted,
                  const LikeGroups *grp = nullptr, const int32_t *chain_bad = nullptr,
                  int32_t *acc_sum = nullptr, int64_t *n_acc = nullptr, bool advance_step = false);


int launch_hyper_logp(beatamd_ctx *ctx, const HyperModel &m, int64_t C, const double *H, const double *llks, double *LL);
constexpr int HYPER_CHAIN_MAX = 1024;
struct HyperChainCall {
    int64_t C = 0, n_steps = 0;
    double *H = nullptr, *LL = nullptr, *scaling = nullptr;
    int32_t *acc_since = nullptr;
    const double *llks = nullptr, *lower = nullptr, *upper = nullptr, *scales = nullptr;
    int kind = 0;
    uint64_t seed = 0, first_chain = 0;
    uint32_t step0 = 0;
    int tune_interval = 0, steps_until_tune = 0, buffer_thinning = 1;
    double *trace = nullptr;
    int64_t *n_acc = nullptr;
};
bool hyper_chain_applicable(int64_t nh, int64_t nterm);
int launch_hyper_chain(beatamd_ctx *ctx, const HyperModel &m, const HyperChainCall &call);

int launch_variance_reduction(beatamd_ctx *ctx, int64_t C, int64_t n, const double *nom, int64_t ld, const double *denom,
                              double *VR);
int launch_standardize(beatamd_ctx *ctx, int64_t C, int64_t T, int64_t N, const double *S, const double *hp, const double *X,
                       double *out);
int launch_ensemble_moments(beatamd_ctx *ctx, int64_t C, int64_t M, const double *X, double *state, int64_t n_seen);
int launch_moments_finish(beatamd_ctx *ctx, int64_t M, const double *state, int64_t n, double *mean, double *std, double *mn,
                          double *mx);
int launch_trace_density(beatamd_ctx *ctx, int64_t E, int64_t T, int64_t N, const double *Y, const double *tmin, double deltat,
                         const double *extent, int64_t ny, int64_t nx, double linewidth, double *grid);

int launch_trace_density(beatamd_ctx *ctx, int64_t E, int64_t T, int64_t N, const double *Y, const double *tmin, double deltat,
                         const double *extent, int64_t ny, int64_t nx, double linewidth, double *grid, const int64_t *ranges);

struct MrComps {
    int64_t off[4];
    int32_t n;
};
constexpr int MR_NT_MAX = 20224;
int launch_moment_magnitude(beatamd_ctx *ctx, int64_t C, int64_t P, const double *Q, int64_t np, const MrComps &comps,
                            const double *k, double *M0, double *Mw);
int launch_moment_rate_span(beatamd_ctx *ctx, const FfiModel &m, int64_t C, const double *Q, const double *st0,
                            const int32_t *chain_bad, double deltat, int64_t *spans);
int launch_moment_rate(beatamd_ctx *ctx, const FfiModel &m, int64_t C, const double *Q, const double *st0, const MrComps &comps,
                       const double *k, double deltat, const int64_t *spans, int64_t kbase, int64_t NT, double *out);

constexpr int GM_HDR = 8, GM_MAX_R = 1024, GM_MAX_N = 2048, GM_MAX_G = 64;
inline int64_t group_moments_stride(int64_t n) { return GM_HDR + n + n * n; }
int launch_group_moments_reset(beatamd_ctx *ctx, int64_t G, int64_t n, double *state, int64_t R, const double *Q, double *ref);
int launch_group_moments_update(beatamd_ctx *ctx, int64_t G, int64_t R, int64_t n, const double *Q, const double *like,
                                int64_t like_stride, const double *ref, double *state);
int launch_group_moments_factor(beatamd_ctx *ctx, int64_t G, int64_t n, const double *state, double *factor, double *cov,
                                int32_t *flags);

int launch_crust_stack(beatamd_ctx *ctx, const double *const *G, int64_t K, int nvar, int64_t P, int64_t Nobs,
                       const double *slips, double *X);
struct PredCovSet {
    int64_t off, n;
    const double *base;
    double *out;
};
int launch_pred_covariance(beatamd_ctx *ctx, int64_t K, int64_t Nobs, const double *X, double *D, int64_t nd, int64_t nmax,
                           const PredCovSet *sets);

struct BallSet {
    int64_t off, n;
};
int launch_ball_rms(beatamd_ctx *ctx, int64_t nd, int64_t nmax, const BallSet *sets, const double *coords, const double *data,
                    double max_dist_perc, double *pmax, double *radius, int32_t *counts, double *stds);

constexpr int SPEC_NTRANS_MIN = 2, SPEC_NTRANS_MAX = 8192;
constexpr int SPEC_WAVE_NTRANS = 512;
int spectrum_check_band(int64_t N, int64_t ntrans, int64_t lo, int64_t hi);
int spectrum_twiddles(beatamd_ctx *ctx, int64_t ntrans, const double **W);
int launch_amp_spectrum(beatamd_ctx *ctx, int64_t R, int64_t N, int64_t xs, int64_t ntrans, int64_t lo, int64_t hi,
                        const double *X, const double *data_spec, int64_t T, double *out);

int launch_gf_tables(beatamd_ctx *ctx, const GfStackCall &call, uint32_t *rowoff, double *fac);
int launch_lsq_seismic(beatamd_ctx *ctx, const SeisLib &lib, int interp, int64_t C, const uint32_t *rowoff, const double *fac,
                       const double *data, int accumulate, double *Nmat, double *b);
int launch_lsq_transpose(beatamd_ctx *ctx, const double *A, double *At, int64_t n);
int launch_lsq_finish(beatamd_ctx *ctx, int64_t C, int64_t P, double *Nmat, double *b, int has_seis, const double *GG,
                      const double *LtL, const double *Ggeo, int64_t Nobs, const double *dgeo, GeoCorr corr, const double *Q,
                      int64_t nparams, int64_t h_off);
constexpr int NNLS_MAX_N = 1024;
// ... 92 lines not shown
```

### beat_amd/csrc/logp.hip

```cpp
#include "kernels.hpp"
#include "metropolis.hpp"

namespace beatamd {

__device__ __forceinline__ double hp_value(const HpSrc &h, int64_t c, int64_t d)
{
    return h.base[c * h.stride + (h.offs ? h.offs[d] : d)];
}

__global__ void __launch_bounds__(256) k_mvn_finish(int64_t C, int64_t nd, int64_t M,
                                                   const double *quad, const double *slog,
                                                   HpSrc hp, double *logpts, int64_t ld)
{
    const int64_t i = (int64_t)blockIdx.x * 256 + threadIdx.x;
    if (i >= C * nd) return;
    const int64_t c = i / nd, d = i - c * nd;
    const double h = hp_value(hp, c, d);
    const double norm = (double)(int16_t)M * (2 * h + LOG_2PI);
    logpts[c * ld + d] = (-0.5) * (slog[d] + norm + (1 / exp(h * 2)) * quad[i]);
}

int launch_mvn_finish(beatamd_ctx *ctx, int64_t C, int64_t nd, int64_t M, const double *quad,
                      const double *slog, HpSrc hp, double *logpts, int64_t ld)
{
    const int64_t n = C * nd;
    if (n == 0) return BEATAMD_OK;
    ScopedTimer tm(ctx, "finish");
    hipLaunchKernelGGL(k_mvn_finish, dim3((unsigned)((n + 255) / 256)), dim3(256), 0, ctx->stream,
                       C, nd, M, quad, slog, hp, logpts, ld);
    BA_HIP(hipGetLastError());
    return BEATAMD_OK;
}

__global__ void __launch_bounds__(256) k_scalar_quad(int64_t C, int64_t nd, int64_t M,
                                                    const double *X, int64_t xs_c, int64_t xs_d,
                                                    const double *w, double *quad)
{
    const int64_t i = (int64_t)blockIdx.x * 4 + (threadIdx.x >> 6);
    const int lane = threadIdx.x & 63;
    if (i >= C * nd) return;
    const int64_t c = i / nd, d = i - c * nd;
    const double *x = X + c * xs_c + d * xs_d;
    const double wd = w[d];
    double q = 0.0;
    for (int64_t k = lane; k < M; k += 64) {
        const double t = wd * x[k];
        q = fma(t, t, q);
    }
    for (int off = 32; off > 0; off >>= 1) q += __shfl_down(q, off, 64);
    if (lane == 0) quad[i] = q;
}

int launch_scalar_quad(beatamd_ctx *ctx, int64_t C, int64_t nd, int64_t M, const double *X,
                       int64_t xs_c, int64_t xs_d, const double *w, double *quad)
{
    const int64_t n = C * nd;
    if (n == 0) return BEATAMD_OK;
    hipLaunchKernelGGL(k_scalar_quad, dim3((unsigned)((n + 3) / 4)), dim3(256), 0, ctx->stream, C,
                       nd, M, X, xs_c, xs_d, w, quad);
    BA_HIP(hipGetLastError());
    return BEATAMD_OK;
}

struct GeoStackArgs {
    const double *G[4];
    ChainVec slips[4];
    int nvar, accumulate;
    int64_t P, Nobs, C;
    double *mu;
};

template <int CH>
__global__ void __launch_bounds__(256) k_geo_stack(GeoStackArgs a)
{
    extern __shared__ __attribute__((aligned(16))) double s_slip[];
    const int64_t c0 = (int64_t)blockIdx.y * CH;
    const int64_t k = (int64_t)blockIdx.x * blockDim.x + threadIdx.x;
    const int64_t P = a.P, Nobs = a.Nobs;
    for (int v = 0; v < a.nvar; v++)
        for (int64_t i = threadIdx.x; i < P * CH; i += blockDim.x) {
            const int64_t p = i / CH, j = i % CH;
            s_slip[v * P * CH + i] = c0 + j < a.C ? a.slips[v].base[(c0 + j) * a.slips[v].stride + a.slips[v].off + p] : 0.0;
        }
    __syncthreads();
    if (k >= Nobs) return;
    double acc[CH];
#pragma unroll
    for (int j = 0; j < CH; j++) acc[j] = (a.accumulate && c0 + j < a.C) ? a.mu[(c0 + j) * Nobs + k] : 0.0;
    for (int v = 0; v < a.nvar; v++) {
        const double *G = a.G[v] + k;
        const double *sl = s_slip + v * P * CH;
        int64_t p = 0;
        double ga[16], gb[16];
        const int64_t nfull = P / 16;
        if (nfull > 0) {
#pragma unroll
            for (int u = 0; u < 16; u++) ga[u] = G[u * Nobs];
        }
        for (int64_t ch = 0; ch < nfull; ch += 2) {
            if (ch + 1 < nfull) {
#pragma unroll
                for (int u = 0; u < 16; u++) gb[u] = G[(p + 16 + u) * Nobs];
// ... 316 lines not shown
```

### beat_amd/csrc/metropolis.hpp

```cpp
#pragma once
#include "kernels.hpp"
#include "philox.hpp"

#define LOG_2PI 1.8378770664093453

#ifdef __HIPCC__
namespace beatamd {

__device__ __forceinline__ bool propose_component(double q0, double delta, double sc, double lo, double up, double &q)
{
    const double d = delta * sc;
    q = q0 + d;
    return q >= lo && q <= up;
}

__device__ __forceinline__ bool metropolis_accept(double beta, double lp, double l0, double log_u)
{
    const double mr = beta * (lp - l0);
    return isfinite(mr) && (log_u < mr);
}

__device__ __forceinline__ double like_serial(const double *l, const LikeGroups &grp, bool bad)
{
    double total = 0.0;
    int k = 0;
    for (int g = 0; g < grp.n; g++) {
        double s = 0.0;
        for (; k < grp.end[g]; k++) s += l[k];
        total += s;
    }
    if (bad) total = __builtin_nan("");
    return total;
}

__device__ __forceinline__ double tune_factor(double acc)
{
    double f = 1.0;
    if (acc < 0.001) f = 0.1;
    else if (acc < 0.05) f = 0.5;
    else if (acc < 0.2) f = 0.9;
    else if (acc > 0.95) f = 10.0;
    else if (acc > 0.75) f = 2.0;
    else if (acc > 0.5) f = 1.1;
    return f;
}

}
#endif
```

### beat_amd/csrc/misfit.hpp

```cpp
#pragma once

#ifdef __HIPCC__
namespace beatamd {

__device__ __forceinline__ bool guard_skips(const int *guard, int want) { return guard && (*guard != 0) != (want != 0); }

__device__ __forceinline__ double band1_y(double w0, double w1, double ri, double rn)
{
    double y = fma(w0, ri, 0.0);
    y = fma(w1, rn, y);
    return y;
}
__device__ __forceinline__ double band1_y(double w0, double ri) { return fma(w0, ri, 0.0); }

template <class Res, class Band>
__device__ __forceinline__ void band1_step(const Res &r, const Band &w, int i, double &ri, double &q)
{
    const double rn = r(i + 1);
    const double y = band1_y(w(i, 0), w(i, 1), ri, rn);
    q = fma(y, y, q);
    ri = rn;
}

struct Band1Tile {
    double q;
    double r_last;
};

template <bool REGS8, int NT, class Res, class Band>
__device__ __forceinline__ Band1Tile band1_tile(const Res &r, const Band &w, int nvalid, bool trace_end)
{
    double q = 0.0, ri = r(0);
    if constexpr (REGS8) {
#pragma unroll
        for (int i0 = 0; i0 < NT; i0 += 8) {
#pragma unroll
            for (int i = i0; i < i0 + 8; i++) {
                if (i + 1 < nvalid) {
                    band1_step(r, w, i, ri, q);
                } else if (i + 1 == nvalid && trace_end) {
                    const double y = band1_y(w(i, 0), ri);
                    q = fma(y, y, q);
                }
            }
            __builtin_amdgcn_sched_barrier(0);
        }
    } else {
        for (int i = 0; i + 1 < nvalid; i++) band1_step(r, w, i, ri, q);
        if (trace_end) {
            const double y = band1_y(w(nvalid - 1, 0), ri);
            q = fma(y, y, q);
        }
    }
    return {q, ri};
}

__device__ __forceinline__ double tile_join(double s, double q_k) { return s + q_k; }
__device__ __forceinline__ double band1_boundary(double s, double yb) { return fma(yb, yb, s); }
__device__ __forceinline__ double band1_join(double s, double q_k, bool has_boundary, double w0, double w1, double r_last,
                                             double r_next_first)
{
    s = tile_join(s, q_k);
    if (has_boundary) s = band1_boundary(s, band1_y(w0, w1, r_last, r_next_first));
    return s;
}

__device__ __forceinline__ double scalar_t(double w, double data, double syn) { return w * (data - syn); }
template <bool REGS8, int NT, class T>
__device__ __forceinline__ double scalar_tile(const T &t, int nvalid)
{
    double q = 0.0;
    if constexpr (REGS8) {
#pragma unroll
        for (int i0 = 0; i0 < NT; i0 += 8) {
#pragma unroll
            for (int i = i0; i < i0 + 8; i++)
                if (i < nvalid) {
                    const double tt = t(i);
                    q = fma(tt, tt, q);
                }
            __builtin_amdgcn_sched_barrier(0);
        }
    } else {
        for (int i = 0; i < nvalid; i++) {
            const double tt = t(i);
            q = fma(tt, tt, q);
        }
    }
    return q;
}

}
#endif
```

### beat_amd/csrc/model.cpp

```cpp
#include "model.hpp"

namespace beatamd {

int wset_quad(beatamd_ctx *ctx, const WeightSet &w, int64_t C, const double *X, int64_t xs_c, int64_t xs_d, double *quad)
{
    if (w.kind == BEATAMD_W_SCALAR)
        return launch_scalar_quad(ctx, C, w.nd, w.M, X, xs_c, xs_d, w.w.get(), quad);
    if (wset_banded(ctx, w))
        return launch_quadform_banded(ctx, w.wb.get(), w.band, w.M, w.nd, C, X, xs_c, xs_d, quad, w.nd);
    QuadformCall q;
    q.A = w.w.get(); q.a_stride = w.M * w.M; q.M = w.M; q.nd = w.nd; q.C = C;
    q.X = X; q.xs_c = xs_c; q.xs_d = xs_d; q.upper_tri = w.upper_tri;
    q.quad = quad; q.q_stride = w.nd;
    return launch_quadform(ctx, q);
}

int64_t model_ndata(const FfiModel &m)
{
    int64_t n = 0;
    for (auto &w : m.wavemaps) n += w.T;
    if (m.has_geo) n += (int64_t)m.geo.sizes.size();
    return n;
}

int64_t model_nterm(const FfiModel &m) { return model_ndata(m) + (m.lap >= 0 ? m.layout.nvar : 0); }

void drop_obs_quads(beatamd_ctx *ctx)
{
    for (auto &m : ctx->models)
        if (m) m->obs_quads_valid = false;
}

int model_check_layout(const FfiModel &m)
{
    const beatamd_ffi_layout &L = m.layout;
    const int64_t np = L.nparams;
    BA_CHECK(np > 0, BEATAMD_EINVAL, "layout: nparams must be positive");
    for (int v = 0; v < L.nvar; v++)
        BA_CHECK(L.slip_off[v] >= 0 && L.slip_off[v] + m.P <= np, BEATAMD_EINVAL, "layout: slip variable %d outside q", v);
    if (!m.wavemaps.empty()) {
        BA_CHECK(L.durations_off >= 0 && L.durations_off + m.P <= np, BEATAMD_EINVAL, "layout: durations outside q");
        BA_CHECK(L.velocities_off >= 0 && L.velocities_off + m.P <= np, BEATAMD_EINVAL, "layout: velocities outside q");
        BA_CHECK(L.nuc_strike_off >= 0 && L.nuc_strike_off + m.nsub <= np && L.nuc_dip_off >= 0 &&
                     L.nuc_dip_off + m.nsub <= np && L.time_off >= 0 && L.time_off + m.nsub <= np,
                 BEATAMD_EINVAL, "layout: hypocentre variables outside q");
    }
    BA_CHECK(!m.wavemaps.empty() || m.has_geo || m.has_pol || m.lap >= 0, BEATAMD_EINVAL, "model has no composite");
    return BEATAMD_OK;
}

int stack_all(beatamd_ctx *ctx, const SeisLib &lib, int64_t C, const double *durations, const double *starttimes,
              const double *slips, int interp, double *out)
{
    GfStackCall k;
    k.libs[0] = &lib; k.nvar = 1; k.interp = interp; k.C = C;
    k.slips[0] = ChainVec{slips, lib.P, 0}; k.durations = ChainVec{durations, lib.P, 0};
    k.st.explicit_st = starttimes; k.mode = GF_STORE_SYN; k.out = out;
    return launch_gfstack(ctx, k);
}

int model_start_times(beatamd_ctx *ctx, const FfiModel &m, int64_t C, const double *Q, double **st0, int32_t **chain_bad)
{
    BA_TRY(ctx->scratch(SL_CHAINBAD, (size_t)C, chain_bad));
    BA_HIP(hipMemsetAsync(*chain_bad, 0, (size_t)C * sizeof(int32_t), ctx->stream));
    BA_TRY(ctx->scratch(SL_ST0, (size_t)C * m.P, st0));
    return launch_sweep_model(ctx, m, Q, C, *st0, *chain_bad);
}

int wavemap_call(beatamd_ctx *ctx, const FfiModel &m, const Wavemap &wm, int64_t C, const double *Q, const double *st0,
                 int32_t *chain_bad, GfStackCall *call)
{
    GfStackCall &k = *call;
    const int64_t np = m.layout.nparams;
    k.nvar = m.layout.nvar;
    for (int v = 0; v < k.nvar; v++) {
        k.libs[v] = get_obj(ctx->seislibs, wm.libs[v]);
        BA_CHECK(k.libs[v] && k.libs[v]->g, BEATAMD_EINVAL, "wavemap refers to a destroyed / empty GF library");
        k.slips[v] = ChainVec{Q, np, m.layout.slip_off[v]};
    }
    k.durations = ChainVec{Q, np, m.layout.durations_off};
    k.st.starttimes0 = st0;
    k.st.Q = Q;
    k.st.nparams = np;
    k.order_key[0] = ChainVec{Q, np, m.layout.nuc_strike_off};
    k.order_key[1] = ChainVec{Q, np, m.layout.nuc_dip_off};
    k.st.shift_off = wm.shift_off.get();
    k.st.nslot = wm.nslot; k.st.tslot = wm.tslot.get(); k.st.slot_shift_off = wm.slot_shift_off.get();
    k.st.chain_bad = chain_bad;
    k.interp = wm.interp;
    k.f32 = wm.f32;
    k.C = C;
    k.data = wm.data.get();
    return BEATAMD_OK;
}

int geo_pole_coefficients(beatamd_ctx *ctx, const Geodetic &g, int64_t C, const double *Q, int64_t np, GeoCorr *gc)
{
    *gc = g.corr;
    if (g.corr.npole == 0 || C == 0) return BEATAMD_OK;
    if (C > g.pole_chains) {
        hipStreamCaptureStatus cap = hipStreamCaptureStatusNone;
        BA_HIP(hipStreamIsCapturing(ctx->stream, &cap));
        BA_CHECK(cap == hipStreamCaptureStatusNone, BEATAMD_EINVAL,
                 "pole coefficients: %lld chains inside a graph capture, the buffer holds %lld (run one step before the capture)",
                 (long long)C, (long long)g.pole_chains);
        BA_HIP(hipStreamSynchronize(ctx->stream));
        g.pole_chains = 0;
        BA_TRY(g.pole_coef.alloc((size_t)C * g.corr.npole * 4));
        g.pole_chains = C;
    }
    gc->pole = g.pole_coef.get();
    return launch_pole_coef(ctx, g.corr.pole_terms, g.corr.npole, Q, np, C, g.pole_coef.get());
}

int geodetic_residual(beatamd_ctx *ctx, const FfiModel &m, int64_t C, const double *Q, double *mu_out, double *res_out)
{
    const Geodetic &g = m.geo;
    const int64_t np = m.layout.nparams;
    if (!Q) {
        BA_HIP(hipMemsetAsync(mu_out, 0, (size_t)g.Nobs * sizeof(double), ctx->stream));
        return launch_geo_residual(ctx, 1, g.Nobs, g.data.get(), g.odws.get(), mu_out, res_out);
    }
    if (m.geo_is_geometry) {
        if (!res_out) return launch_geom_los(ctx, m.geom, Q, np, C, mu_out);
        GeoCorr gc;
        BA_TRY(geo_pole_coefficients(ctx, g, C, Q, np, &gc));
        return launch_geom_los(ctx, m.geom, Q, np, C, nullptr, g.data.get(), g.odws.get(), res_out, gc);
    }
    const GeoLib *gls[4] = {nullptr, nullptr, nullptr, nullptr};
    ChainVec slips[4];
    BA_CHECK(m.layout.nvar <= 4, BEATAMD_EINVAL, "geodetic composite: more than 4 slip variables");
    for (int v = 0; v < m.layout.nvar; v++) {
        gls[v] = get_obj(ctx->geolibs, g.libs[v]);
        BA_CHECK(gls[v], BEATAMD_EINVAL, "geodetic composite refers to a destroyed GF library");
        slips[v] = ChainVec{Q, np, m.layout.slip_off[v]};
    }
    BA_TRY(launch_geo_stack(ctx, gls, m.layout.nvar, C, slips, 0, mu_out));
    if (!res_out) return BEATAMD_OK;
    GeoCorr gc;
    BA_TRY(geo_pole_coefficients(ctx, g, C, Q, np, &gc));
    return launch_geo_residual(ctx, C, g.Nobs, g.data.get(), g.odws.get(), mu_out, res_out, Q, np, gc);
}

int laplacian_quad(beatamd_ctx *ctx, const Laplacian &lap, int64_t C, int64_t nvar, const double *slips, double *quad)
{
    QuadformCall q;
    q.A = lap.L.get(); q.a_stride = 0; q.M = lap.P; q.nd = nvar; q.C = C;
    q.X = slips; q.xs_c = nvar * lap.P; q.xs_d = lap.P;
    q.quad = quad; q.q_stride = nvar;
    return launch_quadform(ctx, q);
}

static int geodetic_wset(beatamd_ctx *ctx, const Geodetic &g, size_t d, WeightSet **ws)
{
    *ws = get_obj(ctx->wsets, g.wsets[d]);
    BA_CHECK(*ws && (*ws)->nd == 1 && (*ws)->M == g.sizes[d], BEATAMD_EINVAL,
             "geodetic dataset %zu: weight set missing or of the wrong size", d);
    return BEATAMD_OK;
}

void polarity_call(const Polarity &p, int64_t C, const double *Q, int64_t np, PolArgs *a)
{
    a->src = p.src; a->nmap = p.nmap; a->ntab = p.ntab; a->NT = p.NT;
    for (int i = 0; i < POL_MAX_MAPS; i++) {
        a->map_end[i] = p.map_end[i]; a->hp_off[i] = p.hp_off[i]; a->hp_fix[i] = p.hp_fix[i];
    }
    a->gamma = p.gamma;
    a->rw = p.rw.get(); a->obs = p.obs.get(); a->utab = p.utab.get(); a->btab = p.btab.get();
    a->Q = Q; a->nparams = np; a->C = C;
}

int ffi_logp_device(beatamd_ctx *ctx, FfiModel &m, int64_t C, const double *Q, double *LL, const LogpOpts &opt)
{
    const int64_t nllk = m.nllk(), nterm = model_nterm(m), np = m.layout.nparams;
    double *const llks = opt.llks;
    BA_CHECK(!(llks && m.has_pol), BEATAMD_EINVAL,
             "the polarity composite has no Gaussian misfit: update_llks / variance reductions are not defined for it "
             "(beat/models/polarity.py defines none)");
    int64_t col = 0, tcol = 0;
    LikeGroups grp;
    double *quad;
    WeightSet *ws;
    int32_t *chain_bad = nullptr;

    if (!m.wavemaps.empty()) {
        double *st0;
        BA_TRY(model_start_times(ctx, m, C, Q, &st0, &chain_bad));
        for (auto &wm : m.wavemaps) {
            ws = get_obj(ctx->wsets, wm.wset);
            BA_CHECK(ws, BEATAMD_EINVAL, "wavemap refers to a destroyed weight set");
            GfStackCall k;
            BA_TRY(wavemap_call(ctx, m, wm, C, Q, st0, chain_bad, &k));
            k.active = opt.active;
            BA_TRY(ctx->scratch(SL_QUAD, (size_t)C * wm.T, &quad));
            if (wm.domain == BEATAMD_DOMAIN_SPECTRUM) {
                double *spec;
                BA_CHECK(ws->nd == wm.T && ws->M == wm.M, BEATAMD_EINVAL, "spectrum wavemap: weight set of the wrong size");
                k.mode = GF_STORE_SYN;
                BA_TRY(ctx->scratch(SL_RESID, (size_t)C * wm.T * wm.N, &k.out));
                BA_TRY(ctx->scratch(SL_SPEC, (size_t)C * wm.T * wm.M, &spec));
                BA_TRY(launch_gfstack(ctx, k));
                BA_TRY(launch_amp_spectrum(ctx, C * wm.T, wm.N, wm.N, wm.ntrans, wm.lo, wm.hi, k.out, wm.data_spec.get(), wm.T,
                                           spec));
                BA_TRY(wset_quad(ctx, *ws, C, spec, wm.T * wm.M, wm.M, quad));
            } else if (ws->kind == BEATAMD_W_SCALAR) {
                k.mode = GF_RESID_SCALAR;
                k.wscalar = ws->w.get();
                k.quad = quad;
                BA_TRY(launch_gfstack(ctx, k));
            } else if (ws->band == 1 && ws->M == wm.N && ws->nd == wm.T && wset_banded(ctx, *ws)) {
                k.mode = GF_RESID_BAND1;
                k.band_w = ws->wb.get();
                k.quad = quad;
                BA_TRY(ctx->scratch(SL_RESID, (size_t)C * wm.T * wm.N, &k.out));
                BA_TRY(launch_gfstack(ctx, k));
            } else {
                k.mode = GF_RESID_STORE;
                BA_TRY(ctx->scratch(SL_RESID, (size_t)C * wm.T * wm.N, &k.out));
                BA_TRY(launch_gfstack(ctx, k));
                BA_TRY(wset_quad(ctx, *ws, C, k.out, wm.T * wm.N, wm.N, quad));
            }
            if (llks)
                BA_TRY(launch_store_misfits(ctx, C, wm.T, quad, llks + tcol, nterm));
            else
                BA_TRY(launch_mvn_finish(ctx, C, wm.T, wm.nsamples(), quad, ws->slog.get(), HpSrc{Q, np, wm.hp_off.get()}, LL + col,
                                         nllk));
            col += wm.T;
            tcol += wm.T;
        }
        grp.end[grp.n++] = (int32_t)col;
    }
    if (m.has_geo) {
        const Geodetic &g = m.geo;
        const size_t nd = g.sizes.size();
        double *mu;
        BA_TRY(ctx->scratch(SL_MU, (size_t)C * g.Nobs * 2, &mu));
        double *res = mu + C * g.Nobs;
        BA_TRY(geodetic_residual(ctx, m, C, Q, mu, res));
        QuadformSmallCall qs;
        bool small = nd <= 8;
        int64_t off = 0;
        for (size_t d = 0; d < nd; d++) {
            BA_TRY(geodetic_wset(ctx, g, d, &ws));
            small = small && ws->kind != BEATAMD_W_SCALAR;
            if (small) {
                qs.A[d] = ws->w.get(); qs.M[d] = ws->M; qs.xoff[d] = off; qs.upper_tri[d] = ws->upper_tri;
                qs.slog[d] = ws->slog.get(); qs.hp_off[d] = g.hp_off.get() + d;
            }
            off += g.sizes[d];
        }
        small = small && quadform_small_applicable((int)nd, qs.M);
        if (small) {
            qs.nd = (int)nd;
            qs.C = C; qs.X = res; qs.xs_c = g.Nobs; qs.Q = Q; qs.nparams = np;
            qs.LL = LL + col; qs.ld = nllk;
            if (llks) {
                qs.LL = llks + tcol; qs.ld = nterm; qs.misfit_only = true;
            }
            BA_TRY(launch_quadform_small(ctx, qs));
        } else {
            BA_TRY(ctx->scratch(SL_QUAD, (size_t)C, &quad));
            off = 0;
            for (size_t d = 0; d < nd; d++) {
                ws = get_obj(ctx->wsets, g.wsets[d]);
                BA_TRY(wset_quad(ctx, *ws, C, res + off, g.Nobs, 0, quad));
                if (llks)
                    BA_TRY(launch_store_misfits(ctx, C, 1, quad, llks + tcol + (int64_t)d, nterm));
                else
                    BA_TRY(launch_mvn_finish(ctx, C, 1, ws->M, quad, ws->slog.get(), HpSrc{Q, np, g.hp_off.get() + d},
                                             LL + col + (int64_t)d, nllk));
                off += g.sizes[d];
            }
        }
        col += (int64_t)nd;
        tcol += (int64_t)nd;
        grp.end[grp.n++] = (int32_t)col;
    }
    if (m.has_pol) {
        PolArgs a;
        polarity_call(m.pol, C, Q, np, &a);
        a.mode = POL_OUT_LLK; a.out = LL + col; a.ld = nllk; a.active = opt.active;
        BA_TRY(launch_polarity(ctx, a));
        col += m.pol.NT;
        grp.end[grp.n++] = (int32_t)col;
    }
    if (m.lap >= 0) {
        Laplacian *lp = get_obj(ctx->laps, m.lap);
        BA_CHECK(lp, BEATAMD_EINVAL, "model refers to a destroyed laplacian");
        const int nvar = m.layout.nvar;
        ChainVec slips[4];
        for (int v = 0; v < nvar; v++) slips[v] = ChainVec{Q, np, m.layout.slip_off[v]};
        double *sl;
        BA_TRY(ctx->scratch(SL_SLIPS, (size_t)C * nvar * lp->P, &sl));
        BA_TRY(launch_gather_slips(ctx, C, nvar, lp->P, slips, sl));
        BA_TRY(ctx->scratch(SL_QUAD, (size_t)C * nvar, &quad));
        BA_TRY(laplacian_quad(ctx, *lp, C, nvar, sl, quad));
        if (llks)
            BA_TRY(launch_store_misfits(ctx, C, nvar, quad, llks + tcol, nterm));
        else
            BA_TRY(launch_laplacian_finish(ctx, C, nvar, lp->P, lp->logdet, quad, HpSrc{Q + m.layout.h_laplacian_off, np, nullptr},
                                           LL + col, nllk));
        col += 1;
        tcol += nvar;
        grp.end[grp.n++] = (int32_t)col;
    }
    BA_CHECK(col == nllk - 1, BEATAMD_EINVAL, "internal: llk layout mismatch");
    if (llks) {
        BA_CHECK(tcol == nterm, BEATAMD_EINVAL, "internal: misfit layout mismatch");
        return launch_misfits_mark_bad(ctx, C, nterm, llks, chain_bad);
// ... 65 lines not shown
    m.lsq_GG.reset();
    if (gl) {
        BA_TRY(m.lsq_GG.alloc((size_t)(P * P)));
        g.A = gl->g.get(); g.B = gl->g.get(); g.lda = gl->Nobs; g.ldb = gl->Nobs; g.K = gl->Nobs; g.O = m.lsq_GG.get();
        BA_TRY(launch_gemm_f64(ctx, g));
    }
    BA_HIP(hipStreamSynchronize(ctx->stream));
    m.lsq_blocks_valid = true;
    return BEATAMD_OK;
}

int lsq_normal_device(beatamd_ctx *ctx, FfiModel &m, int64_t C, const double *Q, double *Nmat, double *b, int32_t **chain_bad)
{
    const int64_t P = m.P, np = m.layout.nparams;
    BA_CHECK(m.lap >= 0, BEATAMD_EINVAL,
             "Least-squares- solution for distributed slip is only available with laplacian regularization!");
    BA_CHECK(m.lsq_var >= 0 && m.lsq_var < m.layout.nvar, BEATAMD_EINVAL,
             "lsq: the model has no inverted slip variable (beatamd_ffi_model_set_lsq_variables)");
    BA_CHECK(!(m.has_geo && m.geo_is_geometry), BEATAMD_EINVAL, "lsq: a geometry-mode geodetic composite is not linear in slip");
    BA_CHECK(!m.has_pol, BEATAMD_EINVAL, "lsq: a model with a polarity composite has no linear slip problem");
    for (auto &wm : m.wavemaps)
        BA_CHECK(wm.domain != BEATAMD_DOMAIN_SPECTRUM, BEATAMD_EINVAL,
                 "lsq: a spectrum-domain wavemap is not linear in slip (the amplitude is taken after the stack)");
    Laplacian *lp = get_obj(ctx->laps, m.lap);
    BA_CHECK(lp && lp->P == P, BEATAMD_EINVAL, "model refers to a destroyed laplacian");
    const GeoLib *gl = nullptr;
    if (m.has_geo) {
        gl = get_obj(ctx->geolibs, m.geo.libs[m.lsq_var]);
        BA_CHECK(gl && gl->P == P, BEATAMD_EINVAL, "geodetic composite refers to a destroyed GF library");
    }
    BA_TRY(lsq_blocks(ctx, m, *lp, gl));
    *chain_bad = nullptr;
    int has_seis = 0;
    if (!m.wavemaps.empty()) {
        double *st0;
        BA_TRY(model_start_times(ctx, m, C, Q, &st0, chain_bad));
        for (auto &wm : m.wavemaps) {
            GfStackCall k;
            BA_TRY(wavemap_call(ctx, m, wm, C, Q, st0, *chain_bad, &k));
            const SeisLib *lib = k.libs[m.lsq_var];
            k.libs[0] = lib;
            uint32_t *rowoff;
            double *fac = nullptr;
            const int nrow = wm.interp == BEATAMD_MULTILINEAR ? 4 : 1;
            BA_TRY(ctx->scratch(SL_ROWOFF, (size_t)(C * lib->T * P * nrow), &rowoff));
            if (nrow == 4) BA_TRY(ctx->scratch(SL_WEIGHTS, (size_t)(C * lib->T * P * 4), &fac));
            BA_TRY(launch_gf_tables(ctx, k, rowoff, fac));
            BA_TRY(launch_lsq_seismic(ctx, *lib, wm.interp, C, rowoff, fac, wm.data.get(), has_seis, Nmat, b));
            has_seis = 1;
        }
    }
    GeoCorr gc;
    if (m.has_geo) BA_TRY(geo_pole_coefficients(ctx, m.geo, C, Q, np, &gc));
    return launch_lsq_finish(ctx, C, P, Nmat, b, has_seis, m.lsq_GG.get(), m.lsq_LtL.get(), gl ? gl->g.get() : nullptr,
                             m.has_geo ? m.geo.Nobs : 0, m.has_geo ? m.geo.data.get() : nullptr, gc, Q, np,
                             m.layout.h_laplacian_off);
}

int draw_multivariate(beatamd_ctx *ctx, int64_t C, int64_t K, int64_t np, const double *factor, int df, uint64_t seed,
                      uint32_t step, uint64_t first_chain, double *delta, double *log_u, int64_t groups)
{
    double *z, *rs = nullptr;
    BA_TRY(ctx->scratch(SL_Z, (size_t)C * K, &z));
    if (df > 0) BA_TRY(ctx->scratch(SL_ROWSCALE, (size_t)C, &rs));
    BA_TRY(launch_philox_normal(ctx, z, C, K, seed, step, first_chain));
    if (log_u || rs) BA_TRY(launch_philox_chain(ctx, C, seed, step, first_chain, df, log_u, rs));
    GemmCall g;
    g.A = z; g.lda = K;
    g.B = factor; g.ldb = np; g.b_kn = 1;
    g.O = delta; g.ldo = np;
    g.M = C; g.N = np; g.K = K;
    g.row_scale = rs;
    if (groups > 1) {
        const int64_t R = C / groups;
        g.M = R; g.nbatch = (int)groups;
        g.sA = R * K; g.sB = K * np; g.sO = R * np; g.sR = R;
    }
    g.timer = "proposal";
    return launch_gemm_f64(ctx, g);
}

static int draw_proposals(beatamd_ctx *ctx, const StepDraw &draw, int64_t C, int64_t np, const double *d_f, const double *d_q0,
                          const double *d_sc, const double *d_lo, const double *d_up, double *qprop, int32_t *inb,
                          const double **lu_out)
{
    const int64_t K = draw.kind < 0 ? draw.K : np;
    double *lu, *de;
    BA_TRY(ctx->scratch(SL_LOGU, (size_t)C, &lu));
    *lu_out = lu;
    if (draw_propose_applicable(K, np))
        return launch_draw_propose(ctx, C, K, np, draw.kind, d_f, draw.df, draw.seed, draw.step, draw.first_chain, d_q0, d_sc,
                                   d_lo, d_up, qprop, lu, inb, draw.groups);
    BA_TRY(ctx->scratch(SL_DELTA, (size_t)C * np, &de));
    if (draw.kind < 0) {
        BA_TRY(draw_multivariate(ctx, C, K, np, d_f, draw.df, draw.seed, draw.step, draw.first_chain, de, lu, draw.groups));
    } else {
        BA_TRY(launch_philox_univariate(ctx, de, C, np, draw.kind, d_f, draw.seed, draw.step, draw.first_chain));
        BA_TRY(launch_philox_chain(ctx, C, draw.seed, draw.step, draw.first_chain, 0, lu, nullptr));
    }
    return launch_propose(ctx, C, np, d_q0, de, d_sc, d_lo, d_up, qprop, inb);
}

int astep_impl(beatamd_ctx *ctx, FfiModel &m, int64_t C, double *Q0, double *L0, const double *delta, const double *scaling,
               const double *lower, const double *upper, const double *log_u, double beta, const double *betas,
               int32_t *accepted, const StepDraw *draw, int32_t *acc_sum, int64_t *n_acc)
{
    BA_CHECK(Q0 && L0 && scaling && lower && upper && accepted && C >= 0 && (draw || (delta && log_u)),
             BEATAMD_EINVAL, "ffi_astep: NULL argument");
    BA_TRY(model_check_layout(m));
    if (C == 0) return BEATAMD_OK;
    const int64_t np = m.layout.nparams, nllk = m.nllk();
    Staging st(ctx);
    const double *d_de = nullptr, *d_sc, *d_lo, *d_up, *d_lu = nullptr, *d_be = nullptr, *d_f = nullptr;
    double *d_q0, *d_l0, *qprop, *lprop;
    int32_t *d_acc;
    BA_TRY(st.out(Q0, (size_t)C * np, &d_q0, true));
    BA_TRY(st.out(L0, (size_t)C * nllk, &d_l0, true));
    BA_TRY(st.out(accepted, (size_t)C, &d_acc));
    BA_TRY(st.in(scaling, (size_t)C, &d_sc));
    BA_TRY(st.in(lower, (size_t)np, &d_lo));
    BA_TRY(st.in(upper, (size_t)np, &d_up));
    if (betas) BA_TRY(st.in(betas, (size_t)C, &d_be));
    BA_TRY(ctx->scratch(SL_QPROP, (size_t)C * np, &qprop));
    BA_TRY(ctx->scratch(SL_LPROP, (size_t)C * nllk, &lprop));
    void *p = nullptr;
    BA_TRY(ctx->get_scratch(SL_MISC, (size_t)C * 4 + 64, &p));
    int32_t *inb = (int32_t *)p;
    if (draw) {
        BA_CHECK(is_device_ptr(Q0) && (!acc_sum || is_device_ptr(acc_sum)) && (!n_acc || is_device_ptr(n_acc)),
                 BEATAMD_EINVAL, "ffi_mstep: chain states and counters live on the device");
        BA_TRY(st.in(draw->factor, (size_t)(draw->kind < 0 ? draw->groups * draw->K * np : np), &d_f));
        BA_TRY(draw_proposals(ctx, *draw, C, np, d_f, d_q0, d_sc, d_lo, d_up, qprop, inb, &d_lu));
    } else {
        BA_TRY(st.in(delta, (size_t)C * np, &d_de));
        BA_TRY(st.in(log_u, (size_t)C, &d_lu));
        BA_TRY(launch_propose(ctx, C, np, d_q0, d_de, d_sc, d_lo, d_up, qprop, inb));
    }
    LikeTail tail;
    const bool fold = nllk * 8 <= 48 * 1024;
    LogpOpts opt;
    opt.tail = fold ? &tail : nullptr;
    opt.active = GfKnobs::get(gf_knobs(ctx).skip_parked, 1) != 0 ? inb : nullptr;
    BA_TRY(ffi_logp_device(ctx, m, C, qprop, lprop, opt));
    BA_TRY(launch_accept(ctx, C, np, nllk, d_q0, d_l0, qprop, lprop, inb, d_lu, beta, d_be, d_acc,
                         fold ? &tail.grp : nullptr, tail.chain_bad, acc_sum, n_acc, draw != nullptr));
    return st.finish();
}

}
```

### beat_amd/csrc/model.hpp

```cpp
#pragma once
#include "kernels.hpp"

namespace beatamd {

template <class T>
T *get_obj(std::vector<std::unique_ptr<T>> &v, int32_t id)
{
    if (id < 0 || (size_t)id >= v.size()) return nullptr;
    return v[id].get();
}

inline bool wset_banded(beatamd_ctx *ctx, const WeightSet &w)
{
    return w.band >= 0 && w.wb && GfKnobs::get(gf_knobs(ctx).qf_band, 1) != 0;
}
int wset_quad(beatamd_ctx *ctx, const WeightSet &w, int64_t C, const double *X, int64_t xs_c, int64_t xs_d, double *quad);

int64_t model_ndata(const FfiModel &m);
int64_t model_nterm(const FfiModel &m);
int model_check_layout(const FfiModel &m);

int stack_all(beatamd_ctx *ctx, const SeisLib &lib, int64_t C, const double *durations, const double *starttimes,
              const double *slips, int interp, double *out);
int model_start_times(beatamd_ctx *ctx, const FfiModel &m, int64_t C, const double *Q, double **st0, int32_t **chain_bad);
int wavemap_call(beatamd_ctx *ctx, const FfiModel &m, const Wavemap &wm, int64_t C, const double *Q, const double *st0,
                 int32_t *chain_bad, GfStackCall *k);
int geodetic_residual(beatamd_ctx *ctx, const FfiModel &m, int64_t C, const double *Q, double *mu_out, double *res_out);
int geo_pole_coefficients(beatamd_ctx *ctx, const Geodetic &g, int64_t C, const double *Q, int64_t np, GeoCorr *gc);
void polarity_call(const Polarity &p, int64_t C, const double *Q, int64_t np, PolArgs *a);
int laplacian_quad(beatamd_ctx *ctx, const Laplacian &lap, int64_t C, int64_t nvar, const double *slips, double *quad);

struct LikeTail {
    LikeGroups grp;
    const int32_t *chain_bad = nullptr;
};
struct LogpOpts {
    LikeTail *tail = nullptr;
    const int32_t *active = nullptr;
    double *llks = nullptr;
};
int ffi_logp_device(beatamd_ctx *ctx, FfiModel &m, int64_t C, const double *Q, double *LL, const LogpOpts &opt = LogpOpts());

int model_obs_quads(beatamd_ctx *ctx, FfiModel &m);
void drop_obs_quads(beatamd_ctx *ctx);

int lsq_normal_device(beatamd_ctx *ctx, FfiModel &m, int64_t C, const double *Q, double *Nmat, double *b, int32_t **chain_bad);

struct StepDraw {
    const double *factor = nullptr;
    int64_t K = 0;
    int32_t kind = -1, df = 0;
    uint64_t seed = 0, first_chain = 0;
    uint32_t step = 0;
    int64_t groups = 1;
};
int draw_multivariate(beatamd_ctx *ctx, int64_t C, int64_t K, int64_t np, const double *factor, int df, uint64_t seed,
                      uint32_t step, uint64_t first_chain, double *delta, double *log_u, int64_t groups = 1);
int astep_impl(beatamd_ctx *ctx, FfiModel &m, int64_t C, double *Q0, double *L0, const double *delta, const double *scaling,
               const double *lower, const double *upper, const double *log_u, double beta, const double *betas,
               int32_t *accepted, const StepDraw *draw = nullptr, int32_t *acc_sum = nullptr, int64_t *n_acc = nullptr);

}
```

### beat_amd/csrc/smc.hip

```cpp
#include "kernels.hpp"
#include "metropolis.hpp"
#include "wave.hpp"

namespace beatamd {

constexpr int SMC_TB = 1024;

__global__ void __launch_bounds__(SMC_TB) k_smc_calc_beta(const double *lik, int64_t stride, int64_t n,
                                                         double beta, double cv, int mode,
                                                         double dbeta, double *out, double *weights)
{
    __shared__ double sh[SMC_TB / 64];
    const int tid = threadIdx.x;
    double m = -INFINITY;
    for (int64_t i = tid; i < n; i += SMC_TB) m = fmax(m, lik[i * stride]);
    const double lmax = block_max_waveorder(m, sh);

    double low = beta, up = 2.0, cur = beta, total = 0.0;
    double step = dbeta;
    bool more = (mode == 1) || (up - low > 1e-6);
    while (more) {
        if (mode == 0) {
            cur = (low + up) / 2.0;
            step = cur - beta;
        }
        double s = 0.0;
        for (int64_t i = tid; i < n; i += SMC_TB) s += exp(step * (lik[i * stride] - lmax));
        total = block_sum_waveorder(s, sh);
        if (mode == 1) break;
        const double mean = total / (double)n;
        double q = 0.0;
        for (int64_t i = tid; i < n; i += SMC_TB) {
            const double d = exp(step * (lik[i * stride] - lmax)) - mean;
            q += d * d;
        }
        const double var = block_sum_waveorder(q, sh) / (double)n;
        const double cov_temp = sqrt(var) / mean;
        if (cov_temp > cv) up = cur; else low = cur;
        more = up - low > 1e-6;
    }
    for (int64_t i = tid; i < n; i += SMC_TB)
        weights[i] = exp(step * (lik[i * stride] - lmax)) / total;
    if (tid == 0) {
        out[0] = cur;
        out[1] = beta;
    }
}

int launch_smc_calc_beta(beatamd_ctx *ctx, int64_t n, const double *lik, int64_t stride, double beta,
                         double cv, int mode, double dbeta, double *out2, double *weights)
{
    ScopedTimer tm(ctx, "stage");
    hipLaunchKernelGGL(k_smc_calc_beta, dim3(1), dim3(SMC_TB), 0, ctx->stream, lik, stride, n, beta,
                       cv, mode, dbeta, out2, weights);
    BA_HIP(hipGetLastError());
    return BEATAMD_OK;
}

__global__ void __launch_bounds__(SMC_TB) k_smc_resample(const double *weights, int64_t n, double aux,
                                                        double *cum, int32_t *idx)
{
    if (threadIdx.x == 0) {
        double c = 0.0;
        int64_t i = 0;
        for (; i + 8 <= n; i += 8) {
            double w[8];
#pragma unroll
            for (int e = 0; e < 8; e++) w[e] = weights[i + e];
#pragma unroll
            for (int e = 0; e < 8; e++) {
                c += w[e];
                cum[i + e] = c;
            }
        }
        for (; i < n; i++) {
            c += weights[i];
            cum[i] = c;
        }
    }
    __threadfence_block();
    __syncthreads();
    for (int64_t i = threadIdx.x; i < n; i += SMC_TB) {
        const double u = ((double)i + aux) / (double)n;
        int64_t lo = 0, hi = n - 1;
// ... 136 lines not shown
    box_muller(r, a, b);
    z[c * K + 2 * j] = a;
    if (2 * j + 1 < K) z[c * K + 2 * j + 1] = b;
}

__global__ void __launch_bounds__(256) k_philox_chain(int64_t C, uint64_t seed, uint32_t step,
                                                     uint64_t first_chain, int df, double *log_u,
                                                     double *row_scale, const uint32_t *step_dev)
{
    if (step_dev) step = *step_dev;
    const int64_t c = (int64_t)blockIdx.x * 256 + threadIdx.x;
    if (c >= C) return;
    const uint32_t gc = (uint32_t)(first_chain + (uint64_t)c), k0 = (uint32_t)seed, k1 = (uint32_t)(seed >> 32);
    if (log_u) log_u[c] = philox_log_u(gc, step, k0, k1);
    if (row_scale) row_scale[c] = philox_t_row_scale(gc, step, df, k0, k1);
}

__global__ void __launch_bounds__(256) k_philox_univariate(double *delta, int64_t C, int64_t np, int kind,
                                                          const double *scale, uint64_t seed, uint32_t step,
                                                          uint64_t first_chain, const uint32_t *step_dev, int *status)
{
    if (step_dev) step = *step_dev;
    const int64_t npair = (np + 1) / 2;
    const int64_t i = (int64_t)blockIdx.x * 256 + threadIdx.x;
    if (i >= C * npair) return;
    const int64_t c = i / npair, j = i - c * npair;
    const uint64_t gc = first_chain + (uint64_t)c;
    const bool second = 2 * j + 1 < np;
    double a, b;
    philox_scaled_pair(kind, (uint32_t)j, (uint32_t)gc, step, (uint32_t)seed, (uint32_t)(seed >> 32), scale[2 * j],
                       second ? scale[2 * j + 1] : 0.0, status, a, b);
    delta[c * np + 2 * j] = a;
    if (second) delta[c * np + 2 * j + 1] = b;
}

int launch_philox_univariate(beatamd_ctx *ctx, double *delta, int64_t C, int64_t np, int kind,
                             const double *scale, uint64_t seed, uint32_t step, uint64_t first_chain)
{
    const int64_t n = C * ((np + 1) / 2);
    if (n == 0) return BEATAMD_OK;
    ScopedTimer tm(ctx, "proposal");
    hipLaunchKernelGGL(k_philox_univariate, dim3((unsigned)((n + 255) / 256)), dim3(256), 0, ctx->stream,
                       delta, C, np, kind, scale, seed, step, first_chain, ctx->step_dev, ctx->d_status);
    BA_HIP(hipGetLastError());
    return BEATAMD_OK;
}

int launch_philox_normal(beatamd_ctx *ctx, double *z, int64_t C, int64_t K, uint64_t seed,
                         uint32_t step, uint64_t first_chain)
{
    const int64_t n = C * ((K + 1) / 2);
    if (n == 0) return BEATAMD_OK;
    hipLaunchKernelGGL(k_philox_normal, dim3((unsigned)((n + 255) / 256)), dim3(256), 0, ctx->stream, z,
                       C, K, seed, step, first_chain, ctx->step_dev);
    BA_HIP(hipGetLastError());
    return BEATAMD_OK;
}

int launch_philox_chain(beatamd_ctx *ctx, int64_t C, uint64_t seed, uint32_t step, uint64_t first_chain,
                        int df, double *log_u, double *row_scale)
{
    if (C == 0) return BEATAMD_OK;
    hipLaunchKernelGGL(k_philox_chain, dim3((unsigned)((C + 255) / 256)), dim3(256), 0, ctx->stream, C,
                       seed, step, first_chain, df, log_u, row_scale, ctx->step_dev);
    BA_HIP(hipGetLastError());
    return BEATAMD_OK;
}

constexpr int DP_CB = 16, DP_MAX = 64;

struct DrawProposeArgs {
    int64_t C, K, np;
    int kind;
    const double *factor;
    int64_t cpg, sF;
    int df;
    uint64_t seed, first_chain;
    uint32_t step;
    const uint32_t *step_dev;
    int *status;
    const double *Q0, *scaling, *lower, *upper;
    double *Qprop, *log_u;
    int32_t *inbounds;
};

__global__ void __launch_bounds__(256) k_draw_propose(DrawProposeArgs a)
{
    __shared__ double Fs[DP_MAX * DP_MAX];
    __shared__ double zs[DP_CB][DP_MAX];
    __shared__ double rs[DP_CB];
    __shared__ int ok[DP_CB];
    const uint32_t step = a.step_dev ? *a.step_dev : a.step;
    const int tid = threadIdx.x;
    const int64_t bpg = (a.cpg + DP_CB - 1) / DP_CB, grp = (int64_t)blockIdx.x / bpg;
    const int64_t c0 = grp * a.cpg + ((int64_t)blockIdx.x - grp * bpg) * DP_CB;
    const int nc = (int)min((int64_t)DP_CB, (grp + 1) * a.cpg - c0);
    const double *factor = a.factor + grp * a.sF;
    const int K = (int)a.K, np = (int)a.np;
    const uint32_t k0 = (uint32_t)a.seed, k1 = (uint32_t)(a.seed >> 32);
    if (a.kind < 0)
        for (int i = tid; i < K * np; i += 256) Fs[i] = factor[i];
    const int npair = (K + 1) / 2;
    for (int i = tid; i < nc * npair; i += 256) {
        const int c = i / npair, j = i - c * npair;
        const uint32_t gc = (uint32_t)(a.first_chain + (uint64_t)(c0 + c));
        double x, y;
        if (a.kind < 0) {
            uint32_t r[4];
            philox4x32_10((uint32_t)j, gc, step, 0u, k0, k1, r);
            box_muller(r, x, y);
        } else {
            philox_scaled_pair(a.kind, (uint32_t)j, gc, step, k0, k1, factor[2 * j],
                               (2 * j + 1 < K) ? factor[2 * j + 1] : 0.0, a.status, x, y);
        }
        zs[c][2 * j] = x;
        if (2 * j + 1 < K) zs[c][2 * j + 1] = y;
    }
    if (tid < nc) {
        const uint32_t gc = (uint32_t)(a.first_chain + (uint64_t)(c0 + tid));
        a.log_u[c0 + tid] = philox_log_u(gc, step, k0, k1);
        rs[tid] = (a.kind < 0 && a.df > 0) ? philox_t_row_scale(gc, step, a.df, k0, k1) : 1.0;
        ok[tid] = 1;
    }
    __syncthreads();
    for (int i = tid; i < nc * np; i += 256) {
        const int c = i / np, n = i - c * np;
        double o;
        if (a.kind < 0) {
            double acc = 0.0;
            for (int k = 0; k < K; k++) acc = fma(zs[c][k], Fs[k * np + n], acc);
            o = (a.df > 0) ? acc * rs[c] : acc;
        } else {
            o = zs[c][n];
        }
        const int64_t g = (c0 + c) * a.np + n;
        double q;
        const bool inside = propose_component(a.Q0[g], o, a.scaling[c0 + c], a.lower[n], a.upper[n], q);
        a.Qprop[g] = q;
        if (!inside) ok[c] = 0;
    }
    __syncthreads();
    for (int i = tid; i < nc * np; i += 256) {
        const int c = i / np;
        if (!ok[c]) {
            const int64_t g = (c0 + c) * a.np + (i - c * np);
            a.Qprop[g] = a.Q0[g];
        }
    }
    if (tid < nc) a.inbounds[c0 + tid] = ok[tid];
}

bool draw_propose_applicable(int64_t K, int64_t np) { return K >= 1 && K <= DP_MAX && np >= 1 && np <= DP_MAX; }

int launch_draw_propose(beatamd_ctx *ctx, int64_t C, int64_t K, int64_t np, int kind, const double *factor,
                        int df, uint64_t seed, uint32_t step, uint64_t first_chain, const double *Q0,
                        const double *scaling, const double *lower, const double *upper, double *Qprop,
                        double *log_u, int32_t *inbounds, int64_t groups)
{
    if (C == 0) return BEATAMD_OK;
    DrawProposeArgs a;
    a.C = C; a.K = K; a.np = np; a.kind = kind; a.factor = factor; a.df = df;
    a.cpg = C / groups; a.sF = groups > 1 ? K * np : 0;
    a.seed = seed; a.first_chain = first_chain; a.step = step; a.step_dev = ctx->step_dev;
    a.status = ctx->d_status;
    a.Q0 = Q0; a.scaling = scaling; a.lower = lower; a.upper = upper;
    a.Qprop = Qprop; a.log_u = log_u; a.inbounds = inbounds;
    ScopedTimer tm(ctx, "proposal");
    hipLaunchKernelGGL(k_draw_propose, dim3((unsigned)(groups * ((a.cpg + DP_CB - 1) / DP_CB))), dim3(256), 0, ctx->stream, a);
    BA_HIP(hipGetLastError());
    return BEATAMD_OK;
}

__global__ void __launch_bounds__(256) k_propose(int64_t C, int64_t nparams, const double *Q0,
                                                const double *delta, const double *scaling,
                                                const double *lower, const double *upper,
                                                double *Qprop, int32_t *inbounds)
{
    const int64_t c = blockIdx.x;
    __shared__ int s_ok;
    if (threadIdx.x == 0) s_ok = 1;
    __syncthreads();
    const double sc = scaling[c];
    int ok = 1;
    for (int64_t k = threadIdx.x; k < nparams; k += 256) {
        double q;
        const bool inside = propose_component(Q0[c * nparams + k], delta[c * nparams + k], sc, lower[k], upper[k], q);
        Qprop[c * nparams + k] = q;
        if (!inside) ok = 0;
    }
    if (!ok) s_ok = 0;
    __syncthreads();
    if (!s_ok)
        for (int64_t k = threadIdx.x; k < nparams; k += 256)
            Qprop[c * nparams + k] = Q0[c * nparams + k];
    if (threadIdx.x == 0) inbounds[c] = s_ok;
}

int launch_propose(beatamd_ctx *ctx, int64_t C, int64_t nparams, const double *Q0,
                   const double *delta, const double *scaling, const double *lower,
                   const double *upper, double *Qprop, int32_t *inbounds)
{
    if (C == 0) return BEATAMD_OK;
    hipLaunchKernelGGL(k_propose, dim3((unsigned)C), dim3(256), 0, ctx->stream, C, nparams, Q0,
                       delta, scaling, lower, upper, Qprop, inbounds);
    BA_HIP(hipGetLastError());
    return BEATAMD_OK;
}

__global__ void __launch_bounds__(256) k_accept(int64_t C, int64_t nparams, int64_t nllk,
                                               double *Q0, double *L0, const double *Qprop,
                                               double *Lprop, const int32_t *inbounds,
                                               const double *log_u, double beta,
                                               const double *betas, int32_t *accepted, LikeGroups grp,
                                               const int32_t *chain_bad, int32_t *acc_sum,
                                               unsigned long long *n_acc, uint32_t *step_dev)
{
    extern __shared__ __attribute__((aligned(16))) double s_l[];
    const int64_t c = blockIdx.x;
    if (!inbounds[c]) {
        if (threadIdx.x == 0) {
            accepted[c] = 0;
            if (step_dev && c == 0) *step_dev += 1u;
        }
        return;
    }
    double lp;
    if (grp.n > 0) {
        for (int64_t k = threadIdx.x; k < nllk - 1; k += 256) s_l[k] = Lprop[c * nllk + k];
        __syncthreads();
        if (threadIdx.x == 0) {
            const double total = like_serial(s_l, grp, chain_bad && chain_bad[c]);
            s_l[nllk - 1] = total;
            Lprop[c * nllk + nllk - 1] = total;
        }
        __syncthreads();
        lp = s_l[nllk - 1];
    } else {
        lp = Lprop[c * nllk + nllk - 1];
    }
    const double b = betas ? betas[c] : beta;
    const bool acc = metropolis_accept(b, lp, L0[c * nllk + nllk - 1], log_u[c]);
    if (acc) {
        for (int64_t k = threadIdx.x; k < nparams; k += 256) Q0[c * nparams + k] = Qprop[c * nparams + k];
        __syncthreads();
        if (grp.n > 0) {
            for (int64_t k = threadIdx.x; k < nllk; k += 256) L0[c * nllk + k] = s_l[k];
        } else {
            for (int64_t k = threadIdx.x; k < nllk; k += 256) L0[c * nllk + k] = Lprop[c * nllk + k];
        }
    }
    if (threadIdx.x == 0) {
        accepted[c] = acc ? 1 : 0;
        if (acc_sum && acc) acc_sum[c] += 1;
        if (n_acc && acc) atomicAdd(n_acc, 1ull);
        if (step_dev && c == 0) *step_dev += 1u;
    }
}

int launch_accept(beatamd_ctx *ctx, int64_t C, int64_t nparams, int64_t nllk, double *Q0,
                  double *L0, const double *Qprop, double *Lprop, const int32_t *inbounds,
                  const double *log_u, double beta, const double *betas, int32_t *accepted,
                  const LikeGroups *grp, const int32_t *chain_bad, int32_t *acc_sum, int64_t *n_acc,
                  bool advance_step)
{
    if (C == 0) return BEATAMD_OK;
    LikeGroups g;
    if (grp) g = *grp;
    const size_t lds = grp ? (size_t)nllk * sizeof(double) : 0;
    BA_CHECK(lds <= 48 * 1024, BEATAMD_EINVAL, "accept: likelihood vector of %lld entries", (long long)nllk);
    ScopedTimer tm(ctx, "astep");
    hipLaunchKernelGGL(k_accept, dim3((unsigned)C), dim3(256), lds, ctx->stream, C, nparams, nllk,
                       Q0, L0, Qprop, Lprop, inbounds, log_u, beta, betas, accepted, g, chain_bad, acc_sum,
                       (unsigned long long *)n_acc, advance_step ? ctx->step_dev : nullptr);
    BA_HIP(hipGetLastError());
    return BEATAMD_OK;
}

__global__ void k_step_advance(uint32_t *step_dev) { *step_dev += 1u; }

int launch_step_advance(beatamd_ctx *ctx)
{
    if (!ctx->step_dev) return BEATAMD_OK;
    hipLaunchKernelGGL(k_step_advance, dim3(1), dim3(1), 0, ctx->stream, ctx->step_dev);
    BA_HIP(hipGetLastError());
    return BEATAMD_OK;
}

}
```

### beat_amd/csrc/sweep.hip

```cpp
#include "kernels.hpp"
#include "wave.hpp"

namespace beatamd {

__device__ __forceinline__ double eq_solve(double a, double b, double f, double h)
{
    double v;
    if (fabs(a - b) >= f * h) {
        v = (a < b) ? a : b;
        v += f * h;
    } else {
        double dab = a - b;
        v = a + b + sqrt(2.0 * f * f * h * h - dab * dab);
        v /= 2.0;
    }
    return v;
}

__device__ __forceinline__ double upwind(const double *t, int i, int j, const double *slow,
                                         double h, int ni, int nj)
{
    int i1 = i - 1, i2 = i + 1, j1 = j - 1, j2 = j + 1;
    if (i1 < 0) i1 = 0;
    if (i2 >= ni) i2 = ni - 1;
// ... 101 lines not shown
        cell(k0, on0, O0, O1, D0, P0);
        fetch(x + sj, k0, on0, O0, D0, P0);
        cell(k1, on1, O1, O2, D1, P1);
        fetch(x + 2 * sj, k1, on1, O1, D1, P1);
        cell(k2, on2, O2, O0, D2, P2);
        x += 3 * sj;
    }
}

__device__ __forceinline__ void sweep_wave(double *t, double *told, const double *slow, const SlowTerms *terms, bool plain, int ni,
                           int nj, double h, int hi, int hj, int lane, bool a_first_version)
{
    const int n = ni * nj;
    for (int k = lane; k < n; k += 64) t[k] = __builtin_inf();
    wave_lds_sync();
    if (lane == 0) t[hi * nj + hj] = 0.0;
    wave_lds_sync();

    double err = 1.0e6;
    int iter = 0;
    while (err > 0.1) {
        for (int k = lane; k < n; k += 64) told[k] = t[k];
        wave_lds_sync();
        for (int sw = 0; sw < 4; sw++) {
            const bool irev = (sw == 1) || (sw == 2);
            const bool jrev = (sw == 2) || (sw == 3);
            if (ni <= 64 && !a_first_version) {
                if (plain)
                    sweep_diag64<true>(t, terms, ni, nj, irev, jrev, lane);
                else
                    sweep_diag64<false>(t, terms, ni, nj, irev, jrev, lane);
                wave_lds_sync();
                continue;
            }
            for (int d = 0; d < ni + nj - 1; d++) {
                for (int base = 0; base < ni; base += 64) {
                    const int ip = base + lane;
                    const int jp = d - ip;
                    if (ip < ni && jp >= 0 && jp < nj) {
                        const int i = irev ? (ni - 1 - ip) : ip;
                        const int j = jrev ? (nj - 1 - jp) : jp;
                        const double v = upwind(t, i, j, slow, h, ni, nj);
                        t[i * nj + j] = v;
                    }
                }
                wave_lds_sync();
            }
        }
        double e = 0.0;
        for (int k = lane; k < n; k += 64) {
            double dlt = t[k] - told[k];
            e += dlt * dlt;
        }
        err = wave_butterfly<OpAdd>(e);
        if (fabs(err - 0.1) <= 1e-9) {
            double es = 0.0;
            for (int k = 0; k < n; k++) {
                double dlt = t[k] - told[k];
                es += dlt * dlt;
            }
            err = es;
        }
        if (++iter >= 100000) break;
    }
}

struct SweepParams {
    int mode;
    int64_t nprob;
    const double *slow;
    const int32_t *hi, *hj;
    int32_t ni, nj;
    double h;
    const double *Q;
    int64_t nparams, vel_off, nuc_strike_off, nuc_dip_off, time_off, P;
    const int32_t *sf_ndip, *sf_nstrike, *sf_off;
    const double *sf_h;
    int32_t nsub;
    double *out;
    int *status;
    int32_t *chain_bad;
    int32_t nmax;
    int32_t first_version;
};

constexpr int SWEEP_TERMS_MAX_CELLS = 5120;
constexpr size_t SWEEP_WG_LDS_DEFAULT = 64 * 1024;

__host__ __device__ inline int sweep_lds_arrays(int nmax) { return nmax <= SWEEP_TERMS_MAX_CELLS ? 4 : 3; }

SweepLdsPlan sweep_lds_plan(int nmax_cells)
{
    SweepLdsPlan pl;
    pl.nmax = (nmax_cells + 1) & ~1;
    const size_t per_wave = (size_t)sweep_lds_arrays(pl.nmax) * pl.nmax * sizeof(double);
    pl.waves = (4 * per_wave <= SWEEP_WG_LDS_DEFAULT) ? 4 : 1;
    pl.bytes = pl.waves * per_wave;
    return pl;
}

template <int WAVES>
__global__ void __launch_bounds__(WAVES * 64) k_fast_sweep(SweepParams a)
{
    extern __shared__ __attribute__((aligned(16))) double smem[];
    const int wave = __builtin_amdgcn_readfirstlane(threadIdx.x >> 6), lane = threadIdx.x & 63;
    const int64_t prob = (int64_t)blockIdx.x * WAVES + wave;
    if (prob >= a.nprob) return;
    const int arrays = sweep_lds_arrays(a.nmax);
    double *t = smem + (size_t)wave * arrays * a.nmax;
    double *told = t + a.nmax;
    double *slow = told + a.nmax;
    SlowTerms *terms = reinterpret_cast<SlowTerms *>(slow);
    const bool first_version = a.first_version != 0 || arrays < 4;
    bool plain = true;

    int ni, nj, hi, hj;
    double h, tadd = 0.0;
    double *out;
    if (a.mode == 0) {
        ni = a.ni;
        nj = a.nj;
        h = a.h;
        hi = a.hi[prob];
        hj = a.hj[prob];
        const double *s = a.slow + prob * (int64_t)(ni * nj);
        if (ni <= 64 && !first_version) {
            for (int k = lane; k < ni * nj; k += 64) plain &= put_terms(terms + k, s[k], h);
        } else {
            for (int k = lane; k < ni * nj; k += 64) slow[k] = s[k];
        }
        out = a.out + prob * (int64_t)(ni * nj);
    } else {
        const int64_t c = prob / a.nsub;
        const int sf = (int)(prob - c * a.nsub);
        ni = a.sf_ndip[sf];
        nj = a.sf_nstrike[sf];
        h = a.sf_h[sf];
        const double *q = a.Q + c * a.nparams;
        const double pd = q[a.nuc_dip_off + sf], ps = q[a.nuc_strike_off + sf];
        hi = (int)(int16_t)(long long)rint((pd - 0.0 - (h / 2.0)) / h);
        hj = (int)(int16_t)(long long)rint((ps - 0.0 - (h / 2.0)) / h);
        tadd = q[a.time_off + sf];
        const double *v = q + a.vel_off + a.sf_off[sf];
        if (ni <= 64 && !first_version) {
            for (int k = lane; k < ni * nj; k += 64) plain &= put_terms(terms + k, 1.0 / v[k], h);
        } else {
            for (int k = lane; k < ni * nj; k += 64) slow[k] = 1.0 / v[k];
        }
        out = a.out + c * a.P + a.sf_off[sf];
    }
    if (hi < 0 || hi >= ni || hj < 0 || hj >= nj) {
        if (lane == 0) {
            atomicOr(a.status, ST_BAD_HYPO);
            if (a.mode == 1 && a.chain_bad) a.chain_bad[prob / a.nsub] = 1;
        }
        hi = min(max(hi, 0), ni - 1);
        hj = min(max(hj, 0), nj - 1);
    }
    wave_lds_sync();
    sweep_wave(t, told, slow, terms, __all(plain) != 0, ni, nj, h, hi, hj, lane, first_version);
    wave_lds_sync();
    for (int k = lane; k < ni * nj; k += 64) out[k] = (a.mode == 0) ? t[k] : (t[k] + tadd);
}

static int launch_sweep(beatamd_ctx *ctx, SweepParams &p, int nmax_cells)
{
    BA_CHECK(nmax_cells > 0 && nmax_cells <= SWEEP_MAX_CELLS, BEATAMD_EINVAL,
             "fast sweep: subfault with %d patches exceeds the LDS-resident limit (%d)",
             nmax_cells, SWEEP_MAX_CELLS);
    const SweepLdsPlan pl = sweep_lds_plan(nmax_cells);
    p.nmax = pl.nmax;
    p.status = ctx->d_status;
    p.first_version = GfKnobs::get(gf_knobs(ctx).sweep_v1, 0) != 0 ? 1 : 0;
    ScopedTimer tm(ctx, "sweep");
    const size_t lds = pl.bytes;
    if (pl.waves == 4) {
        const int W = 4;
        unsigned grid = (unsigned)((p.nprob + W - 1) / W);
        hipLaunchKernelGGL(k_fast_sweep<4>, dim3(grid), dim3(W * 64), lds, ctx->stream, p);
    } else {
        if (lds > SWEEP_WG_LDS_DEFAULT)
            BA_HIP(hipFuncSetAttribute((const void *)k_fast_sweep<1>,
                                       hipFuncAttributeMaxDynamicSharedMemorySize, (int)lds));
        hipLaunchKernelGGL(k_fast_sweep<1>, dim3((unsigned)p.nprob), dim3(64), lds, ctx->stream,
                           p);
    }
    BA_HIP(hipGetLastError());
    return BEATAMD_OK;
}

int launch_sweep_explicit(beatamd_ctx *ctx, const double *slow, double h, const int32_t *hi,
                          const int32_t *hj, int ni, int nj, int64_t C, double *out)
{
    SweepParams p;
    memset(&p, 0, sizeof(p));
    p.mode = 0;
    p.nprob = C;
    p.slow = slow;
    p.hi = hi;
    p.hj = hj;
    p.ni = ni;
    p.nj = nj;
    p.h = h;
    p.out = out;
    return launch_sweep(ctx, p, ni * nj);
}

int launch_sweep_model(beatamd_ctx *ctx, const FfiModel &m, const double *Q, int64_t C,
                       double *starttimes0, int32_t *chain_bad)
{
    SweepParams p;
    memset(&p, 0, sizeof(p));
    p.mode = 1;
    p.nprob = C * m.nsub;
    p.Q = Q;
    p.nparams = m.layout.nparams;
    p.vel_off = m.layout.velocities_off;
    p.nuc_strike_off = m.layout.nuc_strike_off;
    p.nuc_dip_off = m.layout.nuc_dip_off;
    p.time_off = m.layout.time_off;
    p.P = m.P;
    p.sf_ndip = m.d_ndip.get();
    p.sf_nstrike = m.d_nstrike.get();
    p.sf_off = m.d_patch_off.get();
    p.sf_h = m.d_patch_size.get();
    p.nsub = m.nsub;
    p.out = starttimes0;
    p.chain_bad = chain_bad;
    int nmax = 0;
    for (int s = 0; s < m.nsub; s++) nmax = std::max(nmax, m.ndip[s] * m.nstrike[s]);
    return launch_sweep(ctx, p, nmax);
}

}
```

Baseline: 92630 chain-steps/s.

## Fuse per-step kernels: sweep builds GF index tables, step_end folds tile sums

```diff
diff --git a/beat_amd/csrc/ctx.hpp b/beat_amd/csrc/ctx.hpp
--- a/beat_amd/csrc/ctx.hpp
+++ b/beat_amd/csrc/ctx.hpp
@@ -276,7 +276,7 @@
     X(gc_sort, "BEATAMD_GC_SORT") X(gc_keys, "BEATAMD_GC_KEYS") X(gc_bands, "BEATAMD_GC_BANDS") X(gr_cap, "BEATAMD_GR_CAP") \
     X(gr_pass_alloc, "BEATAMD_GR_PASS_ALLOC") X(gr_var, "BEATAMD_GR_VAR") X(sweep_v1, "BEATAMD_SWEEP_V1") X(qf_band, "BEATAMD_QF_BAND") \
     X(qf_fuse, "BEATAMD_QF_FUSE") X(gf_split, "BEATAMD_GF_SPLIT") X(gm_wave, "BEATAMD_GM_WAVE") X(skip_parked, "BEATAMD_SKIP_PARKED") \
-    X(td_strip, "BEATAMD_TD_STRIP") X(pd_strip, "BEATAMD_PD_STRIP") X(pd_rows, "BEATAMD_PD_ROWS")
+    X(td_strip, "BEATAMD_TD_STRIP") X(pd_strip, "BEATAMD_PD_STRIP") X(pd_rows, "BEATAMD_PD_ROWS") X(step_fuse, "BEATAMD_STEP_FUSE")
 struct GfKnobs {
 #define X(member, env) int member = KNOB_UNSET;
     BEATAMD_GF_KNOBS(X)
@@ -327,6 +327,8 @@
     beatamd::GfKnobs knobs;
     bool knobs_live = false;
     uint32_t *step_dev = nullptr;
+    const void *step_sync_p = nullptr;
+    size_t step_sync_cap = 0;
     std::map<int64_t, beatamd::DevMem<double>> twiddles;
 
     int get_scratch(int slot, size_t bytes, void **out);
@@ -362,7 +364,7 @@
     SL_MG_FLAG, SL_MG_MOM, SL_MG_PAR, SL_MG_GRID, SL_MG_W, SL_MG_BOX,
     SL_MC_FLAG, SL_MC_COUNT, SL_MC_SUM, SL_PD_BOX,
     SL_CV_W, SL_CV_SA, SL_CV_SB, SL_CV_Q, SL_CV_CM, SL_CV_RM, SL_CV_OFF, SL_CV_ESS, SL_CV_ACT, SL_CV_STATE, SL_CV_MAC0, SL_CV_MAC1,
-    SL_CV_AC, SL_CV_RHO, SL_CV_PART, SL_COUNT
+    SL_CV_AC, SL_CV_RHO, SL_CV_PART, SL_STEP_SYNC, SL_COUNT
 };
 constexpr int SL_NIN = SL_OUT0 - SL_IN0, SL_NOUT = SL_ROWOFF - SL_OUT0;
 
diff --git a/beat_amd/csrc/gfshared.hip b/beat_amd/csrc/gfshared.hip
--- a/beat_amd/csrc/gfshared.hip
+++ b/beat_amd/csrc/gfshared.hip
@@ -1547,6 +1547,15 @@
     ctx->gs_has_passes = has_passes;
 }
 
+static int sum_tiles_or_leave(beatamd_ctx *ctx, const GfStackCall &k, const double *partial, int ntile, const double *edges)
+{
+    const SeisLib &L = *k.libs[0];
+    if (!k.tiles) return launch_sum_tiles(ctx, partial, k.C * L.T, ntile, k.quad, nullptr, 0, edges, k.band_w, L.T, L.N);
+    k.tiles->partial = partial; k.tiles->edges = edges; k.tiles->band_w = edges ? k.band_w : nullptr;
+    k.tiles->ntile = ntile; k.tiles->T = L.T; k.tiles->N = L.N;
+    return BEATAMD_OK;
+}
+
 static int launch_gfstack_ws(beatamd_ctx *ctx, const GfStackCall &k, const GfPlan &p, const GfLaunch &ln, const GfGroup &g)
 {
     const GfKnobs &kn = *p.knobs;
@@ -1580,7 +1589,9 @@
     BA_TRY(ctx->scratch(SL_GS_W, (size_t)ta.w_var_stride * k.nvar + (size_t)3 * WS_CG, &ta.w));
     {
         ScopedTimer tm(ctx, "grouptables");
-        if (k.active) {
+        if (k.active && k.packed_ready && !ta.order) {
+            ta.order = k.packed_ready;
+        } else if (k.active) {
             uint32_t *packed;
             BA_TRY(ctx->scratch(SL_WS_PACK, (size_t)ngroups * WS_CG, &packed));
             hipLaunchKernelGGL(k_ws_pack, dim3((unsigned)ngroups), dim3(WS_CG), 0, ctx->stream, ta.order, k.active, k.C, packed);
@@ -1638,7 +1649,7 @@
     }
     BA_HIP(hipGetLastError());
     if (a.partial)
-        BA_TRY(launch_sum_tiles(ctx, a.partial, k.C * L.T, a.ntile, k.quad, nullptr, 0, a.edges, k.band_w, L.T, L.N));
+        BA_TRY(sum_tiles_or_leave(ctx, k, a.partial, a.ntile, a.edges));
     return BEATAMD_OK;
 }
 
@@ -1771,7 +1782,7 @@
     ScopedTimer tm(ctx, "gfstack");
     if (ucap_fit) BA_TRY(launch_dma_twin(ctx, k, p, g, a, 1, ucap_fit, ga.windowed, GTP));
     BA_TRY(launch_dma_twin(ctx, k, p, g, a, ucap_fit ? 2 : 0, ucap, ga.windowed, GTP));
-    if (mode == GF_RESID_SCALAR) BA_TRY(launch_sum_tiles(ctx, a.partial, k.C * L.T, a.ntile, k.quad));
+    if (mode == GF_RESID_SCALAR) BA_TRY(sum_tiles_or_leave(ctx, k, a.partial, a.ntile, nullptr));
     return BEATAMD_OK;
 }
 
diff --git a/beat_amd/csrc/gfstack.hip b/beat_amd/csrc/gfstack.hip
--- a/beat_amd/csrc/gfstack.hip
+++ b/beat_amd/csrc/gfstack.hip
@@ -18,14 +18,6 @@
     int64_t R;
 };
 
-__device__ __forceinline__ int to_int16(double x) { return (int)(int16_t)(long long)x; }
-
-__device__ __forceinline__ bool wrap_index(int &i, int n)
-{
-    if (i < 0) i += n;
-    return i >= 0 && i < n;
-}
-
 __global__ void __launch_bounds__(256) k_gf_tables(TabArgs a)
 {
     const int64_t idx = (int64_t)blockIdx.x * 256 + threadIdx.x;
@@ -49,12 +41,7 @@
     const int64_t row0 = (t * a.P + p) * a.D;
     bool ok = true;
     if (a.interp == BEATAMD_NEAREST_NEIGHBOR) {
-        int si = to_int16(rint((st - a.st_min) / a.st_dt));
-        int di = to_int16(rint((du - a.du_min) / a.du_dt));
-        const bool ok_s = wrap_index(si, S), ok_d = wrap_index(di, D);
-        ok = ok_s && ok_d;
-        if (!ok) { si = 0; di = 0; }
-        a.rowoff[idx] = (uint32_t)((row0 + di) * a.S + si);
+        ok = gf_row_nn(GfGrid{a.st_min, a.st_dt, a.du_min, a.du_dt, D, S}, st, du, row0, a.rowoff[idx]);
     } else {
         const double ds = (st - a.st_min) / a.st_dt;
         const double dd = (du - a.du_min) / a.du_dt;
@@ -287,18 +274,7 @@
     const int64_t i = (int64_t)blockIdx.x * 256 + threadIdx.x;
     if (i >= n) return;
     if (guard_skips(guard, want)) return;
-    const int64_t t = edges ? i % T : 0;
-    double s = 0.0;
-    for (int k = 0; k < ntile; k++) {
-        if (edges && k + 1 < ntile) {
-            const double *w = band_w + (t * N + (int64_t)k * 64 + 63) * 2;
-            const double *e = edges + (i * ntile + k) * 2;
-            s = band1_join(s, partial[i * ntile + k], true, w[0], w[1], e[1], e[2]);
-        } else {
-            s = tile_join(s, partial[i * ntile + k]);
-        }
-    }
-    quad[i] = s;
+    quad[i] = tiles_join_row(partial, i, ntile, edges, band_w, edges ? i % T : 0, N);
 }
 
 int launch_sum_tiles(beatamd_ctx *ctx, const double *partial, int64_t n, int ntile, double *quad, const int *guard, int want,
@@ -434,6 +410,13 @@
         p.band1 = gf_band1(false, GF_BY_NONE, &p.mode);
     }
     return p;
+}
+
+bool gf_sweep_tables(const GfStackCall &k, const GfKnobs &kn, int num_cu)
+{
+    if (k.interp != BEATAMD_NEAREST_NEIGHBOR || k.st.explicit_st || !k.st.starttimes0 || k.C == 0) return false;
+    const GfPlan p = gf_plan_call(k, kn, num_cu);
+    return p.tinv && p.R == 1 && p.Ttab == 1 && p.nrow == 1;
 }
 
 static int tune_group_size(beatamd_ctx *ctx, const GfStackCall &k, const GfPlan &p, const GfLaunch &ln, GfGroup *out)
@@ -486,6 +469,7 @@
     SeisLib views[4];
     GfStackCall v = call;
     v.active = nullptr;
+    v.packed_ready = nullptr; v.tiles = nullptr;
     for (int i = 0; i < call.nvar; i++) {
         views[i] = *call.libs[i];
         views[i].T = p.T; views[i].P = p.P;
@@ -563,7 +547,10 @@
     BA_TRY(ctx->scratch(SL_ROWOFF, (size_t)CTP * p.nrow, &ta.rowoff));
     ta.fac = nullptr;
     if (p.nrow == 4) BA_TRY(ctx->scratch(SL_WEIGHTS, (size_t)CTP * 4, &ta.fac));
-    {
+    if (k.tables_ready) {
+        BA_CHECK(k.tables_ready == ta.rowoff && p.tinv && Ttab == 1 && p.nrow == 1, BEATAMD_EINVAL,
+                 "internal: the sweep's index tables are not the ones this plan reads");
+    } else {
         ScopedTimer tm(ctx, "tables");
         hipLaunchKernelGGL(k_gf_tables, dim3((unsigned)((CTP + 255) / 256)), dim3(256), 0,
                            ctx->stream, ta);
diff --git a/beat_amd/csrc/kernels.hpp b/beat_amd/csrc/kernels.hpp
--- a/beat_amd/csrc/kernels.hpp
+++ b/beat_amd/csrc/kernels.hpp
@@ -14,8 +14,9 @@
 SweepLdsPlan sweep_lds_plan(int nmax_cells);
 int launch_sweep_explicit(beatamd_ctx *ctx, const double *slow, double h, const int32_t *hi,
                           const int32_t *hj, int ni, int nj, int64_t C, double *out);
+struct SweepTables;
 int launch_sweep_model(beatamd_ctx *ctx, const FfiModel &m, const double *Q, int64_t C,
-                       double *starttimes0, int32_t *chain_bad);
+                       double *starttimes0, int32_t *chain_bad, const SweepTables *tab = nullptr);
 
 struct StartTimeSrc {
     const double *explicit_st = nullptr;
@@ -43,6 +44,37 @@
 }
 #endif
 
+struct GfGrid {
+    double st_min, st_dt, du_min, du_dt;
+    int D, S;
+};
+#ifdef __HIPCC__
+__device__ __forceinline__ int to_int16(double x) { return (int)(int16_t)(long long)x; }
+
+__device__ __forceinline__ bool wrap_index(int &i, int n)
+{
+    if (i < 0) i += n;
+    return i >= 0 && i < n;
+}
+
+__device__ __forceinline__ bool gf_row_nn(const GfGrid &g, double st, double du, int64_t row0, uint32_t &row)
+{
+    int si = to_int16(rint((st - g.st_min) / g.st_dt));
+    int di = to_int16(rint((du - g.du_min) / g.du_dt));
+    const bool ok_s = wrap_index(si, g.S), ok_d = wrap_index(di, g.D);
+    const bool ok = ok_s && ok_d;
+    if (!ok) { si = 0; di = 0; }
+    row = (uint32_t)((row0 + di) * (int64_t)g.S + si);
+    return ok;
+}
+#endif
+
+struct SweepTables {
+    GfGrid grid;
+    ChainVec durations;
+    uint32_t *rowoff = nullptr;
+};
+
 int gf_patch_ranges(int64_t T, int64_t P, int64_t N, int num_cu);
 
 enum GfMode : int {
@@ -50,6 +82,12 @@
     GF_RESID_SCALAR = 1,
     GF_RESID_STORE = 2,
     GF_RESID_BAND1 = 3
+};
+
+struct TileSums {
+    const double *partial = nullptr, *edges = nullptr, *band_w = nullptr;
+    int ntile = 0;
+    int64_t T = 0, N = 0;
 };
 
 struct GfStackCall {
@@ -69,7 +107,10 @@
     bool f32 = false;
     ChainVec order_key[2];
     const int32_t *active = nullptr;
-};
+    const uint32_t *tables_ready = nullptr, *packed_ready = nullptr;
+    TileSums *tiles = nullptr;
+};
+bool gf_sweep_tables(const GfStackCall &call, const GfKnobs &kn, int num_cu);
 int launch_gfstack(beatamd_ctx *ctx, const GfStackCall &call);
 int launch_sum_tiles(beatamd_ctx *ctx, const double *partial, int64_t n, int ntile, double *quad, const int *guard = nullptr,
                      int want = 0, const double *edges = nullptr, const double *band_w = nullptr, int64_t T = 1, int64_t N = 0);
@@ -322,21 +363,34 @@
 int launch_philox_univariate(beatamd_ctx *ctx, double *delta, int64_t C, int64_t np, int kind,
                              const double *scale, uint64_t seed, uint32_t step, uint64_t first_chain);
 int launch_step_advance(beatamd_ctx *ctx);
+constexpr int STEP_PACK_CG = 512;
+struct StepBegin {
+    int32_t *chain_bad = nullptr;
+    uint32_t *packed = nullptr, *sync = nullptr;
+};
 bool draw_propose_applicable(int64_t K, int64_t np);
+bool draw_propose_packs(int64_t C, int64_t groups);
 int launch_draw_propose(beatamd_ctx *ctx, int64_t C, int64_t K, int64_t np, int kind, const double *factor,
                         int df, uint64_t seed, uint32_t step, uint64_t first_chain, const double *Q0,
                         const double *scaling, const double *lower, const double *upper, double *Qprop,
-                        double *log_u, int32_t *inbounds, int64_t groups = 1);
+                        double *log_u, int32_t *inbounds, int64_t groups = 1, const StepBegin *begin = nullptr);
 int launch_philox_chain(beatamd_ctx *ctx, int64_t C, uint64_t seed, uint32_t step, uint64_t first_chain,
                         int df, double *log_u, double *row_scale);
 int launch_propose(beatamd_ctx *ctx, int64_t C, int64_t nparams, const double *Q0,
                    const double *delta, const double *scaling, const double *lower,
-                   const double *upper, double *Qprop, int32_t *inbounds);
+                   const double *upper, double *Qprop, int32_t *inbounds, const StepBegin *begin = nullptr);
+struct StepEndArgs {
+    TileSums ts;
+    int64_t M = 0;
+    const double *slog = nullptr;
+    HpSrc hp;
+};
 int launch_accept(beatamd_ctx *ctx, int64_t C, int64_t nparams, int64_t nllk, double *Q0,
                   double *L0, const double *Qprop, double *Lprop, const int32_t *inbounds,
                   const double *log_u, double beta, const double *betas, int32_t *accepted,
                   const LikeGroups *grp = nullptr, const int32_t *chain_bad = nullptr,
-                  int32_t *acc_sum = nullptr, int64_t *n_acc = nullptr, bool advance_step = false);
+                  int32_t *acc_sum = nullptr, int64_t *n_acc = nullptr, bool advance_step = false,
+                  const StepEndArgs *end = nullptr);
 
 
 int launch_hyper_logp(beatamd_ctx *ctx, const HyperModel &m, int64_t C, const double *H, const double *llks, double *LL);
diff --git a/beat_amd/csrc/logp.hip b/beat_amd/csrc/logp.hip
--- a/beat_amd/csrc/logp.hip
+++ b/beat_amd/csrc/logp.hip
@@ -2,11 +2,6 @@
 #include "metropolis.hpp"
 
 namespace beatamd {
-
-__device__ __forceinline__ double hp_value(const HpSrc &h, int64_t c, int64_t d)
-{
-    return h.base[c * h.stride + (h.offs ? h.offs[d] : d)];
-}
 
 __global__ void __launch_bounds__(256) k_mvn_finish(int64_t C, int64_t nd, int64_t M,
                                                    const double *quad, const double *slog,
@@ -15,9 +10,7 @@
     const int64_t i = (int64_t)blockIdx.x * 256 + threadIdx.x;
     if (i >= C * nd) return;
     const int64_t c = i / nd, d = i - c * nd;
-    const double h = hp_value(hp, c, d);
-    const double norm = (double)(int16_t)M * (2 * h + LOG_2PI);
-    logpts[c * ld + d] = (-0.5) * (slog[d] + norm + (1 / exp(h * 2)) * quad[i]);
+    logpts[c * ld + d] = mvn_logpt(M, hp_value(hp, c, d), slog[d], quad[i]);
 }
 
 int launch_mvn_finish(beatamd_ctx *ctx, int64_t C, int64_t nd, int64_t M, const double *quad,
diff --git a/beat_amd/csrc/metropolis.hpp b/beat_amd/csrc/metropolis.hpp
--- a/beat_amd/csrc/metropolis.hpp
+++ b/beat_amd/csrc/metropolis.hpp
@@ -18,6 +18,17 @@
 {
     const double mr = beta * (lp - l0);
     return isfinite(mr) && (log_u < mr);
+}
+
+__device__ __forceinline__ double hp_value(const HpSrc &h, int64_t c, int64_t d)
+{
+    return h.base[c * h.stride + (h.offs ? h.offs[d] : d)];
+}
+
+__device__ __forceinline__ double mvn_logpt(int64_t M, double h, double slog, double quad)
+{
+    const double norm = (double)(int16_t)M * (2 * h + LOG_2PI);
+    return (-0.5) * (slog + norm + (1 / exp(h * 2)) * quad);
 }
 
 __device__ __forceinline__ double like_serial(const double *l, const LikeGroups &grp, bool bad)
diff --git a/beat_amd/csrc/misfit.hpp b/beat_amd/csrc/misfit.hpp
--- a/beat_amd/csrc/misfit.hpp
+++ b/beat_amd/csrc/misfit.hpp
@@ -65,6 +65,22 @@
     return s;
 }
 
+__device__ __forceinline__ double tiles_join_row(const double *partial, int64_t i, int ntile, const double *edges,
+                                                 const double *band_w, int64_t t, int64_t N)
+{
+    double s = 0.0;
+    for (int k = 0; k < ntile; k++) {
+        if (edges && k + 1 < ntile) {
+            const double *w = band_w + (t * N + (int64_t)k * 64 + 63) * 2;
+            const double *e = edges + (i * ntile + k) * 2;
+            s = band1_join(s, partial[i * ntile + k], true, w[0], w[1], e[1], e[2]);
+        } else {
+            s = tile_join(s, partial[i * ntile + k]);
+        }
+    }
+    return s;
+}
+
 __device__ __forceinline__ double scalar_t(double w, double data, double syn) { return w * (data - syn); }
 template <bool REGS8, int NT, class T>
 __device__ __forceinline__ double scalar_tile(const T &t, int nvalid)
diff --git a/beat_amd/csrc/model.cpp b/beat_amd/csrc/model.cpp
--- a/beat_amd/csrc/model.cpp
+++ b/beat_amd/csrc/model.cpp
@@ -65,6 +65,24 @@
     BA_HIP(hipMemsetAsync(*chain_bad, 0, (size_t)C * sizeof(int32_t), ctx->stream));
     BA_TRY(ctx->scratch(SL_ST0, (size_t)C * m.P, st0));
     return launch_sweep_model(ctx, m, Q, C, *st0, *chain_bad);
+}
+
+static bool step_fuse(beatamd_ctx *ctx) { return GfKnobs::get(gf_knobs(ctx).step_fuse, 1) != 0; }
+
+static int sweep_for(beatamd_ctx *ctx, const FfiModel &m, int64_t C, const double *Q, double *st0, int32_t *chain_bad,
+                     bool bad_cleared, GfStackCall *k)
+{
+    if (!bad_cleared) BA_HIP(hipMemsetAsync(chain_bad, 0, (size_t)C * sizeof(int32_t), ctx->stream));
+    if (m.wavemaps.size() != 1 || !step_fuse(ctx) || k->libs[0]->P != m.P || !gf_sweep_tables(*k, gf_knobs(ctx), ctx->num_cu))
+        return launch_sweep_model(ctx, m, Q, C, st0, chain_bad);
+    const SeisLib &L = *k->libs[0];
+    BA_CHECK(L.T * L.P * L.D * L.S < (int64_t)0xffffffffLL, BEATAMD_EINVAL, "gfstack: library has more than 2^32 rows");
+    SweepTables tb;
+    tb.grid = GfGrid{L.st_min, L.st_dt, L.du_min, L.du_dt, (int)L.D, (int)L.S};
+    tb.durations = k->durations;
+    BA_TRY(ctx->scratch(SL_ROWOFF, (size_t)(C * L.P), &tb.rowoff));
+    k->tables_ready = tb.rowoff;
+    return launch_sweep_model(ctx, m, Q, C, st0, chain_bad, &tb);
 }
 
 int wavemap_call(beatamd_ctx *ctx, const FfiModel &m, const Wavemap &wm, int64_t C, const double *Q, const double *st0,
@@ -185,13 +203,24 @@
 
     if (!m.wavemaps.empty()) {
         double *st0;
-        BA_TRY(model_start_times(ctx, m, C, Q, &st0, &chain_bad));
+        BA_TRY(ctx->scratch(SL_CHAINBAD, (size_t)C, &chain_bad));
+        BA_TRY(ctx->scratch(SL_ST0, (size_t)C * m.P, &st0));
+        bool swept = false;
+        const auto sweep_and_stack = [&](GfStackCall &k) -> int {
+            if (!swept) BA_TRY(sweep_for(ctx, m, C, Q, st0, chain_bad, opt.bad_cleared, &k));
+            swept = true;
+            return launch_gfstack(ctx, k);
+        };
+        TileSums *const tiles = opt.tail && opt.tail->end && !llks && m.wavemaps.size() == 1 && !m.has_geo && !m.has_pol && m.lap < 0
+                                    ? &opt.tail->end->ts : nullptr;
         for (auto &wm : m.wavemaps) {
             ws = get_obj(ctx->wsets, wm.wset);
             BA_CHECK(ws, BEATAMD_EINVAL, "wavemap refers to a destroyed weight set");
             GfStackCall k;
             BA_TRY(wavemap_call(ctx, m, wm, C, Q, st0, chain_bad, &k));
             k.active = opt.active;
+            k.packed_ready = opt.packed;
+            if (wm.domain != BEATAMD_DOMAIN_SPECTRUM) k.tiles = tiles;
             BA_TRY(ctx->scratch(SL_QUAD, (size_t)C * wm.T, &quad));
             if (wm.domain == BEATAMD_DOMAIN_SPECTRUM) {
                 double *spec;
@@ -199,7 +228,7 @@
                 k.mode = GF_STORE_SYN;
                 BA_TRY(ctx->scratch(SL_RESID, (size_t)C * wm.T * wm.N, &k.out));
                 BA_TRY(ctx->scratch(SL_SPEC, (size_t)C * wm.T * wm.M, &spec));
-                BA_TRY(launch_gfstack(ctx, k));
+                BA_TRY(sweep_and_stack(k));
                 BA_TRY(launch_amp_spectrum(ctx, C * wm.T, wm.N, wm.N, wm.ntrans, wm.lo, wm.hi, k.out, wm.data_spec.get(), wm.T,
                                            spec));
                 BA_TRY(wset_quad(ctx, *ws, C, spec, wm.T * wm.M, wm.M, quad));
@@ -207,24 +236,28 @@
                 k.mode = GF_RESID_SCALAR;
                 k.wscalar = ws->w.get();
                 k.quad = quad;
-                BA_TRY(launch_gfstack(ctx, k));
+                BA_TRY(sweep_and_stack(k));
             } else if (ws->band == 1 && ws->M == wm.N && ws->nd == wm.T && wset_banded(ctx, *ws)) {
                 k.mode = GF_RESID_BAND1;
                 k.band_w = ws->wb.get();
                 k.quad = quad;
                 BA_TRY(ctx->scratch(SL_RESID, (size_t)C * wm.T * wm.N, &k.out));
-                BA_TRY(launch_gfstack(ctx, k));
+                BA_TRY(sweep_and_stack(k));
             } else {
                 k.mode = GF_RESID_STORE;
                 BA_TRY(ctx->scratch(SL_RESID, (size_t)C * wm.T * wm.N, &k.out));
-                BA_TRY(launch_gfstack(ctx, k));
+                BA_TRY(sweep_and_stack(k));
                 BA_TRY(wset_quad(ctx, *ws, C, k.out, wm.T * wm.N, wm.N, quad));
             }
-            if (llks)
+            if (llks) {
                 BA_TRY(launch_store_misfits(ctx, C, wm.T, quad, llks + tcol, nterm));
-            else
+            } else if (tiles && tiles->partial) {
+                StepEndArgs &e = *opt.tail->end;
+                e.M = wm.nsamples(); e.slog = ws->slog.get(); e.hp = HpSrc{Q, np, wm.hp_off.get()};
+            } else {
                 BA_TRY(launch_mvn_finish(ctx, C, wm.T, wm.nsamples(), quad, ws->slog.get(), HpSrc{Q, np, wm.hp_off.get()}, LL + col,
                                          nllk));
+            }
             col += wm.T;
             tcol += wm.T;
         }
@@ -456,7 +489,7 @@
 
 static int draw_proposals(beatamd_ctx *ctx, const StepDraw &draw, int64_t C, int64_t np, const double *d_f, const double *d_q0,
                           const double *d_sc, const double *d_lo, const double *d_up, double *qprop, int32_t *inb,
-                          const double **lu_out)
+                          const double **lu_out, const StepBegin *begin)
 {
     const int64_t K = draw.kind < 0 ? draw.K : np;
     double *lu, *de;
@@ -464,7 +497,7 @@
     *lu_out = lu;
     if (draw_propose_applicable(K, np))
         return launch_draw_propose(ctx, C, K, np, draw.kind, d_f, draw.df, draw.seed, draw.step, draw.first_chain, d_q0, d_sc,
-                                   d_lo, d_up, qprop, lu, inb, draw.groups);
+                                   d_lo, d_up, qprop, lu, inb, draw.groups, begin);
     BA_TRY(ctx->scratch(SL_DELTA, (size_t)C * np, &de));
     if (draw.kind < 0) {
         BA_TRY(draw_multivariate(ctx, C, K, np, d_f, draw.df, draw.seed, draw.step, draw.first_chain, de, lu, draw.groups));
@@ -472,7 +505,20 @@
         BA_TRY(launch_philox_univariate(ctx, de, C, np, draw.kind, d_f, draw.seed, draw.step, draw.first_chain));
         BA_TRY(launch_philox_chain(ctx, C, draw.seed, draw.step, draw.first_chain, 0, lu, nullptr));
     }
-    return launch_propose(ctx, C, np, d_q0, de, d_sc, d_lo, d_up, qprop, inb);
+    return launch_propose(ctx, C, np, d_q0, de, d_sc, d_lo, d_up, qprop, inb, begin);
+}
+
+static int step_pack_buffers(beatamd_ctx *ctx, int64_t C, StepBegin *sb)
+{
+    const int64_t ngroups = (C + STEP_PACK_CG - 1) / STEP_PACK_CG;
+    BA_TRY(ctx->scratch(SL_WS_PACK, (size_t)ngroups * STEP_PACK_CG, &sb->packed));
+    BA_TRY(ctx->scratch(SL_STEP_SYNC, (size_t)ngroups, &sb->sync));
+    const DevBuf &b = ctx->scratch_bufs[SL_STEP_SYNC];
+    if (ctx->step_sync_p != b.p || ctx->step_sync_cap != b.cap) {
+        BA_HIP(hipMemsetAsync(b.p, 0, b.cap, ctx->stream));
+        ctx->step_sync_p = b.p; ctx->step_sync_cap = b.cap;
+    }
+    return BEATAMD_OK;
 }
 
 int astep_impl(beatamd_ctx *ctx, FfiModel &m, int64_t C, double *Q0, double *L0, const double *delta, const double *scaling,
@@ -500,24 +546,38 @@
     void *p = nullptr;
     BA_TRY(ctx->get_scratch(SL_MISC, (size_t)C * 4 + 64, &p));
     int32_t *inb = (int32_t *)p;
+    const bool skip_parked = GfKnobs::get(gf_knobs(ctx).skip_parked, 1) != 0;
+    StepBegin sb;
+    const bool fuse = step_fuse(ctx);
+    if (fuse && !m.wavemaps.empty()) {
+        BA_TRY(ctx->scratch(SL_CHAINBAD, (size_t)C, &sb.chain_bad));
+        const bool packs = !draw || !draw_propose_applicable(draw->kind < 0 ? draw->K : np, np) || draw_propose_packs(C, draw->groups);
+        if (skip_parked && packs) BA_TRY(step_pack_buffers(ctx, C, &sb));
+    }
+    const StepBegin *begin = sb.chain_bad ? &sb : nullptr;
     if (draw) {
         BA_CHECK(is_device_ptr(Q0) && (!acc_sum || is_device_ptr(acc_sum)) && (!n_acc || is_device_ptr(n_acc)),
                  BEATAMD_EINVAL, "ffi_mstep: chain states and counters live on the device");
         BA_TRY(st.in(draw->factor, (size_t)(draw->kind < 0 ? draw->groups * draw->K * np : np), &d_f));
-        BA_TRY(draw_proposals(ctx, *draw, C, np, d_f, d_q0, d_sc, d_lo, d_up, qprop, inb, &d_lu));
+        BA_TRY(draw_proposals(ctx, *draw, C, np, d_f, d_q0, d_sc, d_lo, d_up, qprop, inb, &d_lu, begin));
     } else {
         BA_TRY(st.in(delta, (size_t)C * np, &d_de));
         BA_TRY(st.in(log_u, (size_t)C, &d_lu));
-        BA_TRY(launch_propose(ctx, C, np, d_q0, d_de, d_sc, d_lo, d_up, qprop, inb));
+        BA_TRY(launch_propose(ctx, C, np, d_q0, d_de, d_sc, d_lo, d_up, qprop, inb, begin));
     }
     LikeTail tail;
+    StepEndArgs end;
     const bool fold = nllk * 8 <= 48 * 1024;
     LogpOpts opt;
     opt.tail = fold ? &tail : nullptr;
-    opt.active = GfKnobs::get(gf_knobs(ctx).skip_parked, 1) != 0 ? inb : nullptr;
+    if (fold && fuse) tail.end = &end;
+    opt.active = skip_parked ? inb : nullptr;
+    opt.bad_cleared = sb.chain_bad != nullptr;
+    opt.packed = sb.packed;
     BA_TRY(ffi_logp_device(ctx, m, C, qprop, lprop, opt));
     BA_TRY(launch_accept(ctx, C, np, nllk, d_q0, d_l0, qprop, lprop, inb, d_lu, beta, d_be, d_acc,
-                         fold ? &tail.grp : nullptr, tail.chain_bad, acc_sum, n_acc, draw != nullptr));
+                         fold ? &tail.grp : nullptr, tail.chain_bad, acc_sum, n_acc, draw != nullptr,
+                         end.ts.partial ? &end : nullptr));
     return st.finish();
 }
 
diff --git a/beat_amd/csrc/model.hpp b/beat_amd/csrc/model.hpp
--- a/beat_amd/csrc/model.hpp
+++ b/beat_amd/csrc/model.hpp
@@ -33,11 +33,14 @@
 struct LikeTail {
     LikeGroups grp;
     const int32_t *chain_bad = nullptr;
+    StepEndArgs *end = nullptr;
 };
 struct LogpOpts {
     LikeTail *tail = nullptr;
     const int32_t *active = nullptr;
     double *llks = nullptr;
+    bool bad_cleared = false;
+    const uint32_t *packed = nullptr;
 };
 int ffi_logp_device(beatamd_ctx *ctx, FfiModel &m, int64_t C, const double *Q, double *LL, const LogpOpts &opt = LogpOpts());
 
diff --git a/beat_amd/csrc/smc.hip b/beat_amd/csrc/smc.hip
--- a/beat_amd/csrc/smc.hip
+++ b/beat_amd/csrc/smc.hip
@@ -1,5 +1,6 @@
 #include "kernels.hpp"
 #include "metropolis.hpp"
+#include "misfit.hpp"
 #include "wave.hpp"
 
 namespace beatamd {
@@ -302,7 +303,48 @@
     const double *Q0, *scaling, *lower, *upper;
     double *Qprop, *log_u;
     int32_t *inbounds;
+    StepBegin begin;
 };
+
+__device__ __forceinline__ void step_pack_group(const StepBegin &b, const int32_t *inbounds, int64_t C, int64_t c, int nc)
+{
+    __shared__ int s_last;
+    __shared__ uint32_t s_cnt[STEP_PACK_CG / 64];
+    const int tid = threadIdx.x, lane = tid & 63, wv = tid >> 6;
+    const int64_t g = c / STEP_PACK_CG, c0 = g * STEP_PACK_CG;
+    const uint32_t gsz = (uint32_t)min((int64_t)STEP_PACK_CG, C - c0);
+    __threadfence();
+    __syncthreads();
+    if (tid == 0) {
+        const uint32_t old = atomicAdd(&b.sync[g], (uint32_t)nc);
+        s_last = old + (uint32_t)nc == gsz;
+        if (s_last) b.sync[g] = 0u;
+    }
+    __syncthreads();
+    if (!s_last) return;
+    __threadfence();
+    bool on[2];
+    uint64_t m[2];
+    for (int h = 0; h < 2; h++) {
+        const int q = wv + 4 * h;
+        const int64_t pos = c0 + q * 64 + lane;
+        on[h] = pos < C && __hip_atomic_load(inbounds + pos, __ATOMIC_RELAXED, __HIP_MEMORY_SCOPE_AGENT) != 0;
+        m[h] = __ballot(on[h]);
+        if (lane == 0) s_cnt[q] = (uint32_t)__popcll(m[h]);
+    }
+    __syncthreads();
+    uint32_t total = 0;
+    for (int q = 0; q < STEP_PACK_CG / 64; q++) total += s_cnt[q];
+    uint32_t *o = b.packed + c0;
+    for (int h = 0; h < 2; h++) {
+        const int q = wv + 4 * h;
+        uint32_t before = 0;
+        for (int r = 0; r < q; r++) before += s_cnt[r];
+        if (on[h]) o[before + (uint32_t)__popcll(m[h] & ((1ull << lane) - 1ull))] = (uint32_t)(c0 + q * 64 + lane);
+    }
+    for (int i = tid; i < STEP_PACK_CG; i += 256)
+        if ((uint32_t)i >= total) o[i] = 0xffffffffu;
+}
 
 __global__ void __launch_bounds__(256) k_draw_propose(DrawProposeArgs a)
 {
@@ -367,18 +409,25 @@
             a.Qprop[g] = a.Q0[g];
         }
     }
-    if (tid < nc) a.inbounds[c0 + tid] = ok[tid];
+    if (tid < nc) {
+        a.inbounds[c0 + tid] = ok[tid];
+        if (a.begin.chain_bad) a.begin.chain_bad[c0 + tid] = 0;
+    }
+    if (a.begin.packed) step_pack_group(a.begin, a.inbounds, a.C, c0, nc);
 }
 
 bool draw_propose_applicable(int64_t K, int64_t np) { return K >= 1 && K <= DP_MAX && np >= 1 && np <= DP_MAX; }
+bool draw_propose_packs(int64_t C, int64_t groups) { return groups == 1 || (C / groups) % DP_CB == 0; }
 
 int launch_draw_propose(beatamd_ctx *ctx, int64_t C, int64_t K, int64_t np, int kind, const double *factor,
                         int df, uint64_t seed, uint32_t step, uint64_t first_chain, const double *Q0,
                         const double *scaling, const double *lower, const double *upper, double *Qprop,
-                        double *log_u, int32_t *inbounds, int64_t groups)
+                        double *log_u, int32_t *inbounds, int64_t groups, const StepBegin *begin)
 {
     if (C == 0) return BEATAMD_OK;
     DrawProposeArgs a;
+    if (begin) a.begin = *begin;
+    BA_CHECK(!a.begin.packed || draw_propose_packs(C, groups), BEATAMD_EINVAL, "internal: draw_propose cannot pack these groups");
     a.C = C; a.K = K; a.np = np; a.kind = kind; a.factor = factor; a.df = df;
     a.cpg = C / groups; a.sF = groups > 1 ? K * np : 0;
     a.seed = seed; a.first_chain = first_chain; a.step = step; a.step_dev = ctx->step_dev;
@@ -391,12 +440,10 @@
     return BEATAMD_OK;
 }
 
-__global__ void __launch_bounds__(256) k_propose(int64_t C, int64_t nparams, const double *Q0,
-                                                const double *delta, const double *scaling,
-                                                const double *lower, const double *upper,
-                                                double *Qprop, int32_t *inbounds)
-{
-    const int64_t c = blockIdx.x;
+__device__ __forceinline__ void propose_chain(int64_t c, int64_t nparams, const double *Q0, const double *delta,
+                                              const double *scaling, const double *lower, const double *upper,
+                                              double *Qprop, int32_t *inbounds)
+{
     __shared__ int s_ok;
     if (threadIdx.x == 0) s_ok = 1;
     __syncthreads();
@@ -416,26 +463,49 @@
     if (threadIdx.x == 0) inbounds[c] = s_ok;
 }
 
+__global__ void __launch_bounds__(256) k_propose(int64_t C, int64_t nparams, const double *Q0,
+                                                const double *delta, const double *scaling,
+                                                const double *lower, const double *upper,
+                                                double *Qprop, int32_t *inbounds)
+{
+    propose_chain(blockIdx.x, nparams, Q0, delta, scaling, lower, upper, Qprop, inbounds);
+}
+
+__global__ void __launch_bounds__(256) k_step_begin(int64_t C, int64_t nparams, const double *Q0,
+                                                   const double *delta, const double *scaling,
+                                                   const double *lower, const double *upper,
+                                                   double *Qprop, int32_t *inbounds, StepBegin b)
+{
+    const int64_t c = blockIdx.x;
+    propose_chain(c, nparams, Q0, delta, scaling, lower, upper, Qprop, inbounds);
+    if (b.chain_bad && threadIdx.x == 0) b.chain_bad[c] = 0;
+    if (b.packed) step_pack_group(b, inbounds, C, c, 1);
+}
+
 int launch_propose(beatamd_ctx *ctx, int64_t C, int64_t nparams, const double *Q0,
                    const double *delta, const double *scaling, const double *lower,
-                   const double *upper, double *Qprop, int32_t *inbounds)
+                   const double *upper, double *Qprop, int32_t *inbounds, const StepBegin *begin)
 {
     if (C == 0) return BEATAMD_OK;
-    hipLaunchKernelGGL(k_propose, dim3((unsigned)C), dim3(256), 0, ctx->stream, C, nparams, Q0,
-                       delta, scaling, lower, upper, Qprop, inbounds);
-    BA_HIP(hipGetLastError());
-    return BEATAMD_OK;
-}
-
-__global__ void __launch_bounds__(256) k_accept(int64_t C, int64_t nparams, int64_t nllk,
-                                               double *Q0, double *L0, const double *Qprop,
-                                               double *Lprop, const int32_t *inbounds,
-                                               const double *log_u, double beta,
-                                               const double *betas, int32_t *accepted, LikeGroups grp,
-                                               const int32_t *chain_bad, int32_t *acc_sum,
-                                               unsigned long long *n_acc, uint32_t *step_dev)
-{
-    extern __shared__ __attribute__((aligned(16))) double s_l[];
+    if (begin)
+        hipLaunchKernelGGL(k_step_begin, dim3((unsigned)C), dim3(256), 0, ctx->stream, C, nparams, Q0,
+                           delta, scaling, lower, upper, Qprop, inbounds, *begin);
+    else
+        hipLaunchKernelGGL(k_propose, dim3((unsigned)C), dim3(256), 0, ctx->stream, C, nparams, Q0,
+                           delta, scaling, lower, upper, Qprop, inbounds);
+    BA_HIP(hipGetLastError());
+    return BEATAMD_OK;
+}
+
+template <bool END>
+__device__ __forceinline__ void accept_chain(int64_t C, int64_t nparams, int64_t nllk,
+                                             double *Q0, double *L0, const double *Qprop,
+                                             double *Lprop, const int32_t *inbounds,
+                                             const double *log_u, double beta,
+                                             const double *betas, int32_t *accepted, const LikeGroups &grp,
+                                             const int32_t *chain_bad, int32_t *acc_sum,
+                                             unsigned long long *n_acc, uint32_t *step_dev, const StepEndArgs &e, double *s_l)
+{
     const int64_t c = blockIdx.x;
     if (!inbounds[c]) {
         if (threadIdx.x == 0) {
@@ -446,12 +516,20 @@
     }
     double lp;
     if (grp.n > 0) {
-        for (int64_t k = threadIdx.x; k < nllk - 1; k += 256) s_l[k] = Lprop[c * nllk + k];
+        for (int64_t k = threadIdx.x; k < nllk - 1; k += 256) {
+            if constexpr (END) {
+                const int64_t i = c * (nllk - 1) + k;
+                const double quad = tiles_join_row(e.ts.partial, i, e.ts.ntile, e.ts.edges, e.ts.band_w, k, e.ts.N);
+                s_l[k] = mvn_logpt(e.M, hp_value(e.hp, c, k), e.slog[k], quad);
+            } else {
+                s_l[k] = Lprop[c * nllk + k];
+            }
+        }
         __syncthreads();
         if (threadIdx.x == 0) {
             const double total = like_serial(s_l, grp, chain_bad && chain_bad[c]);
             s_l[nllk - 1] = total;
-            Lprop[c * nllk + nllk - 1] = total;
+            if constexpr (!END) Lprop[c * nllk + nllk - 1] = total;
         }
         __syncthreads();
         lp = s_l[nllk - 1];
@@ -477,11 +555,36 @@
     }
 }
 
+__global__ void __launch_bounds__(256) k_accept(int64_t C, int64_t nparams, int64_t nllk,
+                                               double *Q0, double *L0, const double *Qprop,
+                                               double *Lprop, const int32_t *inbounds,
+                                               const double *log_u, double beta,
+                                               const double *betas, int32_t *accepted, LikeGroups grp,
+                                               const int32_t *chain_bad, int32_t *acc_sum,
+                                               unsigned long long *n_acc, uint32_t *step_dev)
+{
+    extern __shared__ __attribute__((aligned(16))) double s_l[];
+    accept_chain<false>(C, nparams, nllk, Q0, L0, Qprop, Lprop, inbounds, log_u, beta, betas, accepted, grp, chain_bad, acc_sum,
+                        n_acc, step_dev, StepEndArgs(), s_l);
+}
+
+__global__ void __launch_bounds__(256) k_step_end(int64_t C, int64_t nparams, int64_t nllk,
+                                                 double *Q0, double *L0, const double *Qprop,
+                                                 double *Lprop, const int32_t *inbounds, const double *log_u, double beta,
+                                                 const double *betas, int32_t *accepted, LikeGroups grp,
+                                                 const int32_t *chain_bad, int32_t *acc_sum,
+                                                 unsigned long long *n_acc, uint32_t *step_dev, StepEndArgs e)
+{
+    extern __shared__ __attribute__((aligned(16))) double s_l[];
+    accept_chain<true>(C, nparams, nllk, Q0, L0, Qprop, Lprop, inbounds, log_u, beta, betas, accepted, grp, chain_bad, acc_sum,
+                       n_acc, step_dev, e, s_l);
+}
+
 int launch_accept(beatamd_ctx *ctx, int64_t C, int64_t nparams, int64_t nllk, double *Q0,
                   double *L0, const double *Qprop, double *Lprop, const int32_t *inbounds,
                   const double *log_u, double beta, const double *betas, int32_t *accepted,
                   const LikeGroups *grp, const int32_t *chain_bad, int32_t *acc_sum, int64_t *n_acc,
-                  bool advance_step)
+                  bool advance_step, const StepEndArgs *end)
 {
     if (C == 0) return BEATAMD_OK;
     LikeGroups g;
@@ -489,6 +592,15 @@
     const size_t lds = grp ? (size_t)nllk * sizeof(double) : 0;
     BA_CHECK(lds <= 48 * 1024, BEATAMD_EINVAL, "accept: likelihood vector of %lld entries", (long long)nllk);
     ScopedTimer tm(ctx, "astep");
+    if (end) {
+        BA_CHECK(grp && g.n == 1 && g.end[0] == nllk - 1 && end->ts.partial && end->ts.T == nllk - 1, BEATAMD_EINVAL,
+                 "internal: step_end serves a likelihood row that is one wavemap");
+        hipLaunchKernelGGL(k_step_end, dim3((unsigned)C), dim3(256), lds, ctx->stream, C, nparams, nllk,
+                           Q0, L0, Qprop, Lprop, inbounds, log_u, beta, betas, accepted, g, chain_bad, acc_sum,
+                           (unsigned long long *)n_acc, advance_step ? ctx->step_dev : nullptr, *end);
+        BA_HIP(hipGetLastError());
+        return BEATAMD_OK;
+    }
     hipLaunchKernelGGL(k_accept, dim3((unsigned)C), dim3(256), lds, ctx->stream, C, nparams, nllk,
                        Q0, L0, Qprop, Lprop, inbounds, log_u, beta, betas, accepted, g, chain_bad, acc_sum,
                        (unsigned long long *)n_acc, advance_step ? ctx->step_dev : nullptr);
diff --git a/beat_amd/csrc/sweep.hip b/beat_amd/csrc/sweep.hip
--- a/beat_amd/csrc/sweep.hip
+++ b/beat_amd/csrc/sweep.hip
@@ -207,6 +207,9 @@
     int32_t *chain_bad;
     int32_t nmax;
     int32_t first_version;
+    uint32_t *tab_rowoff;
+    GfGrid tab_grid;
+    ChainVec tab_dur;
 };
 
 constexpr int SWEEP_TERMS_MAX_CELLS = 5120;
@@ -285,6 +288,23 @@
     wave_lds_sync();
     sweep_wave(t, told, slow, terms, __all(plain) != 0, ni, nj, h, hi, hj, lane, first_version);
     wave_lds_sync();
+    if (a.mode == 1 && a.tab_rowoff) {
+        const int64_t c = prob / a.nsub;
+        const int64_t p0 = a.sf_off[(int)(prob - c * a.nsub)];
+        const double *du = a.tab_dur.base + c * a.tab_dur.stride + a.tab_dur.off + p0;
+        uint32_t *row = a.tab_rowoff + c * a.P + p0;
+        bool ok = true;
+        for (int k = lane; k < ni * nj; k += 64) {
+            const double st = t[k] + tadd;
+            out[k] = st;
+            ok &= gf_row_nn(a.tab_grid, st, du[k], (p0 + k) * (int64_t)a.tab_grid.D, row[k]);
+        }
+        if (!ok) {
+            atomicOr(a.status, ST_INDEX_OOB);
+            if (a.chain_bad) a.chain_bad[c] = 1;
+        }
+        return;
+    }
     for (int k = lane; k < ni * nj; k += 64) out[k] = (a.mode == 0) ? t[k] : (t[k] + tadd);
 }
 
@@ -332,11 +352,14 @@
 }
 
 int launch_sweep_model(beatamd_ctx *ctx, const FfiModel &m, const double *Q, int64_t C,
-                       double *starttimes0, int32_t *chain_bad)
+                       double *starttimes0, int32_t *chain_bad, const SweepTables *tab)
 {
     SweepParams p;
     memset(&p, 0, sizeof(p));
     p.mode = 1;
+    if (tab) {
+        p.tab_rowoff = tab->rowoff; p.tab_grid = tab->grid; p.tab_dur = tab->durations;
+    }
     p.nprob = C * m.nsub;
     p.Q = Q;
     p.nparams = m.layout.nparams;
```

Result: no change. 92470 chain-steps/s (-0.2%).
